# kason-huang/StreamVLN

Measured on AMD Instinct MI355X. Metric: action-steps/sec (8-frame window, StreamVLN-Qwen-1.5), higher is better.
Workload: dtype bf16

## Files before the change

include/streamvln_hip.h:

```cpp
#ifndef STREAMVLN_HIP_H
#define STREAMVLN_HIP_H

#include <stdint.h>

#ifdef __cplusplus
extern "C" {
#endif

typedef struct svln_engine svln_engine;

enum { SVLN_BF16 = 0, SVLN_F32 = 1 };

typedef struct svln_config {
    int32_t v_hidden, v_inter, v_heads, v_layers, v_patch, v_image;
    float v_eps;
    int32_t hidden, layers, q_heads, kv_heads, head_dim, inter, vocab;
    float rope_theta, rms_eps;
    int32_t max_positions;
    int32_t max_envs;
    int32_t max_frames;
    int32_t dtype;
} svln_config;

int svln_create(const svln_config* cfg, int device, svln_engine** out);
// ... 164 lines not shown
int svln_op_gemv_fp8(svln_engine* h, const void* w8, const float* scale, int ldw, const void* x, const void* norm_w, float eps, const void* bias,
                     const void* res, void* y, int N, int K, int epi, int32_t* host_token);
int svln_op_quant_mxfp4(svln_engine* h, const void* w_bf16, int64_t rows, int cols, void* q4, void* e8);
int svln_op_gemv_mxfp4(svln_engine* h, const void* q4, const void* e8, int ldw, const void* x, const void* norm_w, float eps, const void* bias,
                       const void* res, void* y, int N, int K, int epi, int32_t* host_token);
int svln_op_pack_rows(svln_engine* h, const void* w_bf16, int ldw, int64_t rows, int cols, void* packed, void* records, int64_t* fallback_blocks);
int svln_op_unpack_rows(svln_engine* h, const void* packed, const void* records, const void* w_bf16, int ldw, int64_t rows, int cols, void* out);
int svln_op_gemv_packed(svln_engine* h, const void* packed, const void* records, const void* W, int ldw, const void* x, const void* norm_w, float eps,
                        const void* bias, const void* res, void* y, int N, int K, int epi, int32_t* host_token);
int svln_op_gemv_mxfp4_batched(svln_engine* h, const void* q4, const void* e8, int ldw, const void* x, int ldx, const void* bias, const void* res,
                               int ldr, void* y, int ldy, int N, int K, int epi, int B, int32_t* host_tokens);
int svln_op_gemv_mxfp4_batched_argmax_pen(svln_engine* h, const void* q4, const void* e8, int ldw, const void* x, int ldx, int N, int K, int B,
                                          const void* pen_flags, const int32_t* pen_rows, float penalty, int32_t* host_tokens);
int svln_op_gemv_argmax_scores(svln_engine* h, int fmt, const void* W, const void* aux, int ldw, const void* x, int N, int K, const void* pen_flags,
                               float penalty, int32_t* host_token, float* host_logprob);
int svln_op_gemv_argmax_topk(svln_engine* h, int fmt, const void* W, const void* aux, int ldw, const void* x, int N, int K, const void* pen_flags,
                             float penalty, int k, int sampled, float temperature, uint64_t seed, int32_t stream, int32_t draw, int32_t* host_token,
                             float* host_logprob, float* part_val, int32_t* part_idx, float* part_sum, float* part_raw, float* part_max,
                             float* cand_val, int32_t* cand_idx, int32_t* top_ids, float* top_logprobs, int32_t* n_part);
int svln_op_gemv_batched_argmax_topk(svln_engine* h, const void* W, int ldw, const void* x, int ldx, int N, int K, int B, const void* pen_flags,
                                     const int32_t* pen_rows, float penalty, int k, int sampled, float temperature, uint64_t seed, const int32_t* streams,
                                     const int32_t* draws, int32_t* host_tokens, float* host_logprobs, float* cand_val, int32_t* cand_idx,
                                     int32_t* top_ids, float* top_logprobs, int32_t* n_part);
int svln_op_gemm_argmax_topk(svln_engine* h, const void* A, int lda, const void* W, int ldw, int M, int N, int K, const void* pen_flags,
                             const int32_t* pen_rows, float penalty, int k, int sampled, float temperature, uint64_t seed, const int32_t* streams,
                             const int32_t* draws, int32_t* host_tokens, float* host_logprobs, float* cand_val, int32_t* cand_idx, int32_t* top_ids,
                             float* top_logprobs, int32_t* n_part);
int svln_op_truncate(svln_engine* h, const float* cand_val, const int32_t* cand_idx, int B, int n_part, int c, const int32_t* streams,
                     const int32_t* draws, uint64_t seed, float temperature, int32_t top_k, float top_p, float* part_val, int32_t* part_idx,
                     float* part_raw, float* part_max, float* part_sum, int32_t* host_tokens, float* host_logprobs);
int svln_op_gemv_batched_argmax_scores(svln_engine* h, const void* W, int ldw, const void* x, int ldx, const void* norm_w, float eps, int N, int K, int B,
                                       const void* pen_flags, const int32_t* pen_rows, float penalty, int32_t* host_tokens, float* host_logprobs);
int svln_op_gemm_argmax_scores(svln_engine* h, const void* A, int lda, const void* W, int ldw, int M, int N, int K, const void* pen_flags,
                               const int32_t* pen_rows, float penalty, int32_t* host_tokens, float* host_logprobs);
int svln_op_gemv_batched_target(svln_engine* h, const void* W, int ldw, const void* x, int ldx, int N, int K, int B, const int32_t* targets, float inv_t,
                                int32_t* host_tokens, float* host_greedy_logprobs, float* host_logprobs, float* host_slots);
int svln_op_gemm_target(svln_engine* h, const void* A, int lda, const void* W, int ldw, int M, int N, int K, const int32_t* targets, float inv_t,
                        int32_t* host_tokens, float* host_greedy_logprobs, float* host_logprobs, float* host_slots);
int svln_op_read_argmax_partials(svln_engine* h, int rows, int n, float* val, int32_t* idx, float* sum);
int svln_op_gemv_argmax_sample(svln_engine* h, int fmt, const void* W, const void* aux, int ldw, const void* x, int N, int K, const void* pen_flags,
                               float penalty, float temperature, uint64_t seed, int32_t stream, int32_t draw, int32_t* host_token, float* host_logprob);
int svln_op_gemv_batched_argmax_sample(svln_engine* h, const void* W, int ldw, const void* x, int ldx, const void* norm_w, float eps, int N, int K, int B,
                                       const void* pen_flags, const int32_t* pen_rows, float penalty, float temperature, uint64_t seed,
                                       const int32_t* streams, const int32_t* draws, int32_t* host_tokens, float* host_logprobs);
int svln_op_gemm_argmax_sample(svln_engine* h, const void* A, int lda, const void* W, int ldw, int M, int N, int K, const void* pen_flags,
                               const int32_t* pen_rows, float penalty, float temperature, uint64_t seed, const int32_t* streams,
                               const int32_t* draws, int32_t* host_tokens, float* host_logprobs);
int svln_op_gumbel(svln_engine* h, uint64_t seed, int32_t stream, int32_t draw, int32_t n0, int32_t count, float* host_out);
int svln_op_subset_argmax(svln_engine* h, const void* W, int ldw, const void* x, int ldx, int V, int K, int B, const int64_t* ids, int n,
                          const void* pen_flags, const int32_t* pen_rows, float penalty, float temperature, uint64_t seed, const int32_t* streams,
                          const int32_t* draws, int32_t* host_tokens, float* host_logprobs, float* host_y, float* host_dist);
int svln_op_rmsnorm(svln_engine* h, const void* x, const void* g, void* y, int rows, int n, float eps);
int svln_op_layernorm(svln_engine* h, const void* x, const void* g, const void* b, void* y, int rows, int n, float eps);
int svln_op_rmsnorm_tap(svln_engine* h, const void* x, const void* g, void* y, int rows, int n, float eps, int skip_value, void* y2, int y2_row_value,
                        int y2_cap);
int svln_op_rmsnorm_indexed(svln_engine* h, const void* x, int x_rows, const void* g, void* y, const int32_t* src_rows, const int32_t* tap_rows,
                            void* tap, int tap_cap, int rows, int n, float eps);
int svln_op_gather_rows(svln_engine* h, const int32_t* src, int rows, const void* embed, int embed_rows, const void* feats, int feat_rows, void* out,
                        int n, int skip_value);
int svln_op_gather_rows_ragged(svln_engine* h, const int32_t* list, int rows, const void* embed, int embed_rows, void* out, int out_rows, int n);
int svln_op_frame_hash(svln_engine* h, const void* pix_dev, int F, int64_t words_per_frame, uint64_t* out_keys);
int svln_op_attention_llm(svln_engine* h, void* qkv, int ld, int T, int P, const void* ctx_qkv, int ctx_T, void* out, int o_stride,
                          int nsplit);
int svln_op_attention_vit(svln_engine* h, const void* qkv, int ld, int F, void* out, int o_stride);
int svln_op_attention_decode(svln_engine* h, int B, const void* ctx_qkv, int ld, int64_t ctx_rows, const int32_t* pos, const void* qkv_new,
                             void* out, int o_stride);
int svln_op_attention_verify(svln_engine* h, int rows, const void* ctx_qkv, int ld, int ctx_rows, const void* qkv_new, void* out,
                             int o_stride);
int svln_op_attention_verify_multi(svln_engine* h, int n_seq, int rows_max, const void* ctx_qkv, int ld, int ctx_rows, const int32_t* ctx_len,
                                   const void* qkv_new, const int32_t* rows, int share, void* out, int o_stride);
int svln_op_verify_step(svln_engine* h, int rows, const int32_t* fed, const int32_t* cand, int count, int max_new, const int64_t* eos,
                        int n_eos, int32_t* new_count, int32_t* done, int64_t* emitted, int32_t* next_token);
int svln_op_kv_read(svln_engine* h, int env, int start, int n, float* k_out, float* v_out);
int svln_op_kv_pool_read(svln_engine* h, int layer, int start, int n, float* k_out, float* v_out);
int svln_op_kv_page_copy(svln_engine* h, int src_page, const int32_t* dst_pages, int n_dst);
int svln_op_beam_page_gather(svln_engine* h, const int32_t* src_pages, const int32_t* dst_pages, int n);
int svln_op_beam_select(svln_engine* h, int W, int limit, int B, int n_cp, int len_cap, const int32_t* eos, int n_eos, const int32_t* list_ids,
                        const float* list_lps, const int32_t* hdr_in, const float* score_in, const int32_t* ids_in, const float* lps_in,
                        const int32_t* set_pages, int32_t* hdr_out, float* score_out, int32_t* ids_out, float* lps_out, int32_t* tok_b,
                        int32_t* pair_src, int32_t* pair_dst, int32_t* rec);
int svln_op_llm_qkv_rope(svln_engine* h, const void* x, int T, int P, void* q_out, int q_stride, int32_t* fused);
int svln_op_set_pages(svln_engine* h, int env, const int32_t* pages, int n);
int svln_op_fill_attn_state(svln_engine* h, float pool_value, int part_nan);
int svln_op_vit_qkv_attention(svln_engine* h, int layer, const void* x, int F, void* qkv_out, void* attn_out, int o_stride,
                              int force_split, int32_t* packer);
int svln_op_fill_vit_state(svln_engine* h, float pool_value, int part_nan);
int svln_op_vit_kv_read(svln_engine* h, float* k_out, float* v_out);
int svln_op_pool(svln_engine* h, const void* in, void* out, int F);
int svln_op_patchify(svln_engine* h, const float* pix, void* out, int F);

#ifdef __cplusplus
}
#endif
#endif
```

streamvln_amd/_lib.py:

```python
from __future__ import annotations

import ctypes as C
import os

_HERE = os.path.dirname(os.path.abspath(__file__))
LIB_PATH = os.environ.get("SVLN_LIB") or os.path.join(_HERE, "libstreamvln_hip.so")

SVLN_BF16, SVLN_F32 = 0, 1
EPI_NONE, EPI_GELU_TANH, EPI_GELU_ERF, EPI_SWIGLU, EPI_ARGMAX = 0, 1, 2, 3, 4


class SvlnConfig(C.Structure):
    _fields_ = [
        ("v_hidden", C.c_int32), ("v_inter", C.c_int32), ("v_heads", C.c_int32), ("v_layers", C.c_int32),
        ("v_patch", C.c_int32), ("v_image", C.c_int32), ("v_eps", C.c_float),
        ("hidden", C.c_int32), ("layers", C.c_int32), ("q_heads", C.c_int32), ("kv_heads", C.c_int32),
        ("head_dim", C.c_int32), ("inter", C.c_int32), ("vocab", C.c_int32),
        ("rope_theta", C.c_float), ("rms_eps", C.c_float),
        ("max_positions", C.c_int32), ("max_envs", C.c_int32), ("max_frames", C.c_int32), ("dtype", C.c_int32),
    ]


class SvlnTurnArgs(C.Structure):
    _fields_ = [
# ... 140 lines not shown
    "svln_op_decode_layer": (_I, [_P, C.POINTER(SvlnDecodeLayerOp)]),
    "svln_decode_layer_supported": (_I, [_I, _I, _I, _I, _I, _I, _PI32]),
    "svln_decode_layer_walk": (_I, [C.POINTER(SvlnDecodeLayerWalkOp), C.POINTER(SvlnDecodeLayerWalkOp), _I, _I, C.POINTER(SvlnDecodeLayerSlot), _I,
                                    _PI32, _PI64]),
    "svln_set_fp8_decode": (_I, [_P, _I]),
    "svln_set_fp8_gemm": (_I, [_P, _I]),
    "svln_set_fp8_scaled_mfma": (_I, [_P, _I]),
    "svln_set_mxfp4_decode": (_I, [_P, _I]),
    "svln_set_mxfp4_batched": (_I, [_P, _I]),
    "svln_set_packed_decode": (_I, [_P, _I]),
    "svln_packed_stats": (_I, [_P, _PI64, _PI64, _PI64, _PI64]),
    "svln_op_pack_rows": (_I, [_P, _P, _I, _I64, _I, _P, _P, _PI64]),
    "svln_op_unpack_rows": (_I, [_P, _P, _P, _P, _I, _I64, _I, _P]),
    "svln_op_gemv_packed": (_I, [_P, _P, _P, _P, _I, _P, _P, _F, _P, _P, _P, _I, _I, _I, _PI32]),
    "svln_set_speculative": (_I, [_P, _I]),
    "svln_set_draft": (_I, [_P, _I, _PI64, _I]),
    "svln_draft_stats": (_I, [_P, _PI64, _PI64, _PI64, _I]),
    "svln_set_prefill_draft": (_I, [_P, _I]),
    "svln_prefill_draft_stats": (_I, [_P, _PI64, _PI64, _PI64, _I]),
    "svln_set_batch_draft": (_I, [_P, _I]),
    "svln_batch_draft_stats": (_I, [_P, _PI64, _PI64, _PI64, _PI64, _PI64, _I]),
    "svln_set_memory_prune": (_I, [_P, _I]),
    "svln_op_memory_prune": (_I, [_P, _P, _I, _I, _PI32, _PF]),
    "svln_probe_reset": (_I, [_P]),
    "svln_probe_read": (_I, [_P, _PD, _PI64, _PD]),
    "svln_probe_read_prefill": (_I, [_P, _PD, _PI64, _PD, _PD, _PD]),
    "svln_phase_times": (_I, [_P, _PD, _PD, _PD, _I]),
    "svln_set_feature_cache": (_I, [_P, _I]),
    "svln_feature_cache_stats": (_I, [_P, _PI64, _PI64]),
    "svln_op_gemm": (_I, [_P, _P, _I, _P, _I, _P, _I, _P, _P, _I, _I, _I, _I, _I, _I, _I, _I]),
    "svln_op_gemm_norm": (_I, [_P, _P, _I, _P, _I, _P, _I, _P, _P, _I, _P, _P, _P, _F, _I, _I, _I, _I, _PI32]),
    "svln_op_gemm_norm_q8": (_I, [_P, _P, _I, _P, _I, _P, _I, _P, _I, _P, _P, _F, _I, _I, _I, _I, _P, _P, _PI32]),
    "svln_gemm_plan": (_I, [C.POINTER(SvlnGemmProblem), C.POINTER(SvlnGemmPlan)]),
    "svln_op_gemv": (_I, [_P, _P, _I, _P, _P, _F, _P, _P, _P, _I, _I, _I, _PI32]),
    "svln_op_gemm_fp8": (_I, [_P, _P, _P, _I, _P, _P, _I, _P, _I, _P, _P, _I, _I, _I, _I, _I, _I, _I]),
    "svln_op_gemv_batched": (_I, [_P, _P, _I, _P, _I, _P, _F, _P, _P, _I, _P, _I, _I, _I, _I, _I, _PI32]),
    "svln_op_quant_fp8": (_I, [_P, _P, _I64, _I, _P, _P]),
    "svln_op_gemv_fp8": (_I, [_P, _P, _P, _I, _P, _P, _F, _P, _P, _P, _I, _I, _I, _PI32]),
    "svln_op_quant_mxfp4": (_I, [_P, _P, _I64, _I, _P, _P]),
    "svln_op_gemv_mxfp4": (_I, [_P, _P, _P, _I, _P, _P, _F, _P, _P, _P, _I, _I, _I, _PI32]),
    "svln_op_gemv_mxfp4_batched": (_I, [_P, _P, _P, _I, _P, _I, _P, _P, _I, _P, _I, _I, _I, _I, _I, _PI32]),
    "svln_op_gemv_mxfp4_batched_argmax_pen": (_I, [_P, _P, _P, _I, _P, _I, _I, _I, _I, _P, _P, _F, _PI32]),
    "svln_op_gemv_argmax_scores": (_I, [_P, _I, _P, _P, _I, _P, _I, _I, _P, _F, _PI32, _PF]),
    "svln_op_gemv_argmax_topk": (_I, [_P, _I, _P, _P, _I, _P, _I, _I, _P, _F, _I, _I, _F, _U64, _I, _I, _PI32, _PF, _PF, _PI32, _PF, _PF, _PF,
                                      _PF, _PI32, _PI32, _PF, _PI32]),
    "svln_op_gemv_batched_argmax_scores": (_I, [_P, _P, _I, _P, _I, _P, _F, _I, _I, _I, _P, _P, _F, _PI32, _PF]),
    "svln_op_gemm_argmax_scores": (_I, [_P, _P, _I, _P, _I, _I, _I, _I, _P, _P, _F, _PI32, _PF]),
    "svln_op_gemv_argmax_sample": (_I, [_P, _I, _P, _P, _I, _P, _I, _I, _P, _F, _F, _U64, _I, _I, _PI32, _PF]),
    "svln_op_gemv_batched_argmax_sample": (_I, [_P, _P, _I, _P, _I, _P, _F, _I, _I, _I, _P, _P, _F, _F, _U64, _PI32, _PI32, _PI32, _PF]),
    "svln_op_gemm_argmax_sample": (_I, [_P, _P, _I, _P, _I, _I, _I, _I, _P, _P, _F, _F, _U64, _PI32, _PI32, _PI32, _PF]),
    "svln_op_gumbel": (_I, [_P, _U64, _I, _I, _I, _I, _PF]),
    "svln_op_subset_argmax": (_I, [_P, _P, _I, _P, _I, _I, _I, _I, _PI64, _I, _P, _P, _F, _F, _U64, _PI32, _PI32, _PI32, _PF, _PF, _PF]),
    "svln_op_rmsnorm": (_I, [_P, _P, _P, _P, _I, _I, _F]),
    "svln_op_layernorm": (_I, [_P, _P, _P, _P, _P, _I, _I, _F]),
    "svln_op_rmsnorm_tap": (_I, [_P, _P, _P, _P, _I, _I, _F, _I, _P, _I, _I]),
    "svln_op_rmsnorm_indexed": (_I, [_P, _P, _I, _P, _P, _PI32, _PI32, _P, _I, _I, _I, _F]),
    "svln_op_gather_rows": (_I, [_P, _PI32, _I, _P, _I, _P, _I, _P, _I, _I]),
    "svln_op_gather_rows_ragged": (_I, [_P, _PI32, _I, _P, _I, _P, _I, _I]),
    "svln_op_frame_hash": (_I, [_P, _P, _I, _I64, C.POINTER(C.c_uint64)]),
    "svln_op_attention_llm": (_I, [_P, _P, _I, _I, _I, _P, _I, _P, _I, _I]),
    "svln_op_attention_vit": (_I, [_P, _P, _I, _I, _P, _I]),
    "svln_op_attention_decode": (_I, [_P, _I, _P, _I, _I64, _PI32, _P, _P, _I]),
    "svln_op_attention_verify": (_I, [_P, _I, _P, _I, _I, _P, _P, _I]),
    "svln_op_attention_verify_multi": (_I, [_P, _I, _I, _P, _I, _I, _PI32, _P, _PI32, _I, _P, _I]),
    "svln_op_verify_step": (_I, [_P, _I, _PI32, _PI32, _I, _I, _PI64, _I, _PI32, _PI32, _PI64, _PI32]),
    "svln_op_kv_read": (_I, [_P, _I, _I, _I, _PF, _PF]),
    "svln_op_llm_qkv_rope": (_I, [_P, _P, _I, _I, _P, _I, _PI32]),
    "svln_op_set_pages": (_I, [_P, _I, _PI32, _I]),
    "svln_op_fill_attn_state": (_I, [_P, _F, _I]),
    "svln_op_vit_qkv_attention": (_I, [_P, _I, _P, _I, _P, _P, _I, _I, _PI32]),
    "svln_op_fill_vit_state": (_I, [_P, _F, _I]),
    "svln_op_vit_kv_read": (_I, [_P, _PF, _PF]),
    "svln_op_pool": (_I, [_P, _P, _P, _I]),
    "svln_op_patchify": (_I, [_P, _P, _P, _I]),
}

_lib = None


def load():
    global _lib
    if _lib is None:
        if not os.path.exists(LIB_PATH):
            raise RuntimeError(f"{LIB_PATH} is missing: build it with streamvln_amd/csrc/build.sh "
                               f"(or __graft_entry__.build()); there is no fallback path")
        import torch
        lib = C.CDLL(LIB_PATH)
        for name, (res, args) in SIGNATURES.items():
            fn = getattr(lib, name)
            fn.restype, fn.argtypes = res, args
        _lib = lib
    return _lib


class SvlnError(RuntimeError):
    pass


def check(rc: int):
    if rc != 0:
        raise SvlnError(load().svln_last_error().decode("utf-8", "replace"))
```

streamvln_amd/csrc/attention.hip:

```cpp
#include <type_traits>

#include "common.h"
#include "kernels.h"

namespace svln {

namespace {

template <typename T, int HD> struct AttnGeom {
    static constexpr int EPC = Elt<T>::PER_CHUNK;
    static constexpr int HDC = (((HD + EPC - 1) / EPC) + 1) & ~1;
    static constexpr int HDP = HDC * EPC;
    static constexpr int DT = (HD + 31) / 32;
    static constexpr int VROWS = DT * 32;
    static constexpr int VC = 64 / EPC;
    static constexpr bool KSWZ = (HDC % 16) == 0;
    static constexpr int KROW = (KSWZ ? HDC : HDC + 1) * 16;
    static constexpr int K_TILE_BYTES = 64 * KROW;
    static constexpr int V_TILE_BYTES = VROWS * VC * 16;
};

SVLN_DEV float fast_exp2(float x) { return __builtin_amdgcn_exp2f(x); }

template <typename G> SVLN_DEV int k_off(int row, int c) {
    return row * G::KROW + ((G::KSWZ ? (c ^ (row & 15)) : c) << 4);
}
SVLN_DEV int v_off_f32(int row, int c) { return row * 256 + ((c ^ (row & 15)) << 4); }
SVLN_DEV int v_off_bf16(int row, int unit) { return row * 128 + ((unit ^ ((row >> 1) & 15)) << 3); }

template <int OFF> SVLN_DEV void lds_read_b64(uint2& v, unsigned addr) { asm volatile("ds_read_b64 %0, %1 offset:%2" : "=v"(v) : "v"(addr), "n"(OFF)); }
template <int N> SVLN_DEV void lds_wait(uint2& a, uint2& b) { asm volatile("s_waitcnt lgkmcnt(%2)" : "+v"(a), "+v"(b) : "n"(N)); }
template <int I, int N, typename F> SVLN_DEV void static_for(F&& f) {
    if constexpr (I < N) { f(std::integral_constant<int, I>{}); static_for<I + 1, N>(f); }
}

template <typename T, int HD, int WAVES, int KG = 1, int PF = 1>
__global__ __launch_bounds__(WAVES * 64 * KG, (KG == 1 && WAVES == 4 && sizeof(T) == 2) ? 2 : 1) void attn_kernel(AttnArgs p) {
    using G = AttnGeom<T, HD>;
    constexpr int NT = WAVES * 64;
    constexpr int EPC = G::EPC;
    extern __shared__ __attribute__((aligned(16))) char smem[];
    const int kg = KG == 1 ? 0 : (int)threadIdx.x / NT;
    char* sK = smem + kg * (G::K_TILE_BYTES + G::V_TILE_BYTES);
    char* sV = sK + G::K_TILE_BYTES;

    const int tid = KG == 1 ? (int)threadIdx.x : (int)threadIdx.x - kg * NT, lane = tid & 63, wave = tid >> 6;
    const int r = lane & 31, h = lane >> 5;
    const int kh = blockIdx.y;
    const int frame = kh / p.hpf, head0 = (kh % p.hpf) * p.G;
    const int kt0 = blockIdx.z * p.tiles_per_split + kg;
    const int page0 = p.page_table ? p.page_table[kt0] : kt0;
    const int kv_len = p.dyn_kv_len ? *p.dyn_kv_len : p.kv_len;
    const int P = p.dyn_kv_len ? kv_len - p.T : p.P;
    const int rows_total = p.T * p.G;
    const int rho = (blockIdx.x * WAVES + wave) * 32 + r;
    const bool valid = rho < rows_total;
    const int qi = valid ? rho / p.G : 0;
    const int qg = valid ? rho - qi * p.G : 0;
    const int qpos = P + qi;

    uint4 qf[G::HDC / 2];
    {
        const T* qrow = (const T*)p.Q + (size_t)(frame * p.T + qi) * p.q_stride + (size_t)(head0 + qg) * HD;
#pragma unroll
        for (int s = 0; s < G::HDC / 2; ++s) {
            const int e0 = (2 * s + h) * EPC;
            qf[s] = (valid && e0 < HD) ? *(const uint4*)(qrow + e0) : zero_chunk();
        }
    }
    int tiles = (kv_len + 63) >> 6;
    if (p.causal) {
        const int last_row = min((int)(blockIdx.x + 1) * WAVES * 32, rows_total) - 1;
        const int last_pos = P + last_row / p.G;
        tiles = min(tiles, (last_pos >> 6) + 1);
    }
    const int kt_begin = blockIdx.z * p.tiles_per_split + kg;
    const int kt_end = min(tiles, (int)blockIdx.z * p.tiles_per_split + p.tiles_per_split);
    const int n_iter = (kt_end - (int)blockIdx.z * p.tiles_per_split + KG - 1) / KG;

    const float scale2 = p.scale * 1.4426950408889634f;
    f32x16 O[G::DT];
#pragma unroll
    for (int d = 0; d < G::DT; ++d)
#pragma unroll
        for (int e = 0; e < 16; ++e) O[d][e] = 0.0f;
    float m = -INFINITY, l = 0.0f;

    const size_t k_page_stride = (size_t)p.n_kv_total * 64 * G::HDP * sizeof(T);
    const size_t v_page_stride = (size_t)p.n_kv_total * G::VROWS * 64 * sizeof(T);

    constexpr bool PFK = WAVES == 4 || (KG > 1 && PF >= 1), PFV = WAVES == 4 || (KG > 1 && PF == 1);
    constexpr int KTOT = 64 * G::HDC, VTOT = G::VROWS * G::VC, B = WAVES == 1 ? 4 : 8;
    constexpr int KL = (KTOT + NT - 1) / NT, VL = (VTOT + NT - 1) / NT;
    uint4 pk[PFK ? KL : 1], pv[PFV ? VL : 1];
    auto tile_ptrs = [&](int kt, const char*& gk, const char*& gv) {
        const int pg = kt == kt0 ? page0 : (p.page_table ? p.page_table[kt] : kt);
        gk = (const char*)p.Kpool + (size_t)pg * k_page_stride + (size_t)kh * 64 * G::HDP * sizeof(T);
        gv = (const char*)p.Vpool + (size_t)pg * v_page_stride + (size_t)kh * G::VROWS * 64 * sizeof(T);
    };
    auto put_k = [&](int q, const uint4& v) {
        const int row = q / G::HDC, c = q - row * G::HDC;
        *(uint4*)(sK + k_off<G>(row, c)) = v;
    };
    auto put_v = [&](int q, const uint4& v) {
        const int row = q / G::VC, c = q - row * G::VC;
        if (sizeof(T) == 4) {
            *(uint4*)(sV + v_off_f32(row, c)) = v;
        } else {
            *(uint2*)(sV + v_off_bf16(row, 2 * c)) = make_uint2(v.x, v.y);
            *(uint2*)(sV + v_off_bf16(row, 2 * c + 1)) = make_uint2(v.z, v.w);
        }
    };
    auto load_regs = [&](int kt) {
        const char *gk, *gv;
        tile_ptrs(kt, gk, gv);
        if (PFK) {
#pragma unroll
            for (int u = 0; u < KL; ++u) {
                const int q = tid + u * NT;
                pk[u] = q < KTOT ? *(const uint4*)(gk + (size_t)q * 16) : zero_chunk();
            }
        }
        if (PFV) {
#pragma unroll
            for (int u = 0; u < VL; ++u) {
                const int q = tid + u * NT;
                pv[u] = q < VTOT ? *(const uint4*)(gv + (size_t)q * 16) : zero_chunk();
            }
        }
    };
    if (PFK && kt_begin < kt_end) load_regs(kt_begin);
// ... 18 lines not shown
                    for (int u = 0; u < B; ++u) {
                        const int q = tid + (b0 + u) * NT;
                        t[u] = (b0 + u < KL && q < KTOT) ? *(const uint4*)(gK + (size_t)q * 16) : zero_chunk();
                    }
#pragma unroll
                    for (int u = 0; u < B; ++u) {
                        const int q = tid + (b0 + u) * NT;
                        if (b0 + u < KL && q < KTOT) put_k(q, t[u]);
                    }
                }
            }
            if (PFV) {
#pragma unroll
                for (int u = 0; u < VL; ++u) {
                    const int q = tid + u * NT;
                    if (q < VTOT) put_v(q, pv[u]);
                }
            } else {
#pragma unroll
                for (int b0 = 0; b0 < VL; b0 += B) {
                    uint4 t[B];
#pragma unroll
                    for (int u = 0; u < B; ++u) {
                        const int q = tid + (b0 + u) * NT;
                        t[u] = (b0 + u < VL && q < VTOT) ? *(const uint4*)(gV + (size_t)q * 16) : zero_chunk();
                    }
#pragma unroll
                    for (int u = 0; u < B; ++u) {
                        const int q = tid + (b0 + u) * NT;
                        if (b0 + u < VL && q < VTOT) put_v(q, t[u]);
                    }
                }
            }
        }
        __syncthreads();
        if (PFK && kt + KG < kt_end) load_regs(kt + KG);
        if (act) {

        f32x16 S[2];
#pragma unroll
        for (int j = 0; j < 2; ++j)
#pragma unroll
            for (int e = 0; e < 16; ++e) S[j][e] = 0.0f;
#pragma unroll
        for (int s = 0; s < G::HDC / 2; ++s) {
#pragma unroll
            for (int j = 0; j < 2; ++j) {
                const uint4 a = *(const uint4*)(sK + k_off<G>(j * 32 + r, 2 * s + h));
                mma_chunk<T>(a, qf[s], S[j]);
            }
        }

        const int tile_last_key = kt * 64 + 63;
        const bool need_mask = tile_last_key >= kv_len || (p.causal && tile_last_key > P + (int)(blockIdx.x * WAVES * 32) / p.G);
        if (need_mask) {
#pragma unroll
            for (int j = 0; j < 2; ++j)
#pragma unroll
                for (int e = 0; e < 16; ++e) {
                    const int key = kt * 64 + j * 32 + acc_row(e, lane);
                    if (!(key < kv_len && (!p.causal || key <= qpos))) S[j][e] = -INFINITY;
                }
        }
        float mloc = -INFINITY;
#pragma unroll
        for (int j = 0; j < 2; ++j)
#pragma unroll
            for (int e = 0; e < 16; ++e) mloc = fmaxf(mloc, S[j][e]);
        mloc = fmaxf(mloc, __shfl_xor(mloc, 32, 64)) * scale2;
        const float mnew = fmaxf(m, mloc);
        float alpha = 1.0f, psum = 0.0f;
        if (mnew == -INFINITY) {
#pragma unroll
            for (int j = 0; j < 2; ++j)
#pragma unroll
                for (int e = 0; e < 16; ++e) S[j][e] = 0.0f;
        } else {
            alpha = fast_exp2(m - mnew);
#pragma unroll
            for (int j = 0; j < 2; ++j)
#pragma unroll
                for (int e = 0; e < 16; ++e) {
                    const float pv = fast_exp2(fmaf(S[j][e], scale2, -mnew));
                    S[j][e] = pv;
                    psum += pv;
                }
        }
        l = l * alpha + psum;
        m = mnew;
        if (__builtin_amdgcn_ballot_w64(alpha != 1.0f) != 0) {
#pragma unroll
            for (int d = 0; d < G::DT; ++d)
#pragma unroll
                for (int e = 0; e < 16; ++e) O[d][e] *= alpha;
        }

        if (sizeof(T) == 2) {
            const unsigned sv0 = (unsigned)(size_t)(__attribute__((address_space(3))) char*)sV + r * 128;
            const int xr = (r >> 1) & 15;
#pragma unroll
            for (int ks = 0; ks < 4; ++ks) {
                const int j = ks >> 1, b0 = 8 * (ks & 1);
                const unsigned alo = sv0 + (((4 * ks + h) ^ xr) << 3), ahi = sv0 + (((4 * ks + 2 + h) ^ xr) << 3);
                uint2 vlo[G::DT], vhi[G::DT];
                static_for<0, G::DT>([&](auto dc) {
                    constexpr int d = decltype(dc)::value;
                    lds_read_b64<d * 4096>(vlo[d], alo);
// ... 8 lines not shown
                                                                   __builtin_bit_cast(bf16x8, pf), O[d], 0, 0, 0);
                });
            }
        } else {
#pragma unroll
            for (int j = 0; j < 2; ++j)
#pragma unroll
                for (int g4 = 0; g4 < 4; ++g4) {
#pragma unroll
                    for (int d = 0; d < G::DT; ++d) {
                        const uint4 a = *(const uint4*)(sV + v_off_f32(d * 32 + r, j * 8 + 2 * g4 + h));
                        O[d] = __builtin_amdgcn_mfma_f32_32x32x2f32(__uint_as_float(a.x), S[j][4 * g4 + 0], O[d], 0, 0, 0);
                        O[d] = __builtin_amdgcn_mfma_f32_32x32x2f32(__uint_as_float(a.y), S[j][4 * g4 + 1], O[d], 0, 0, 0);
                        O[d] = __builtin_amdgcn_mfma_f32_32x32x2f32(__uint_as_float(a.z), S[j][4 * g4 + 2], O[d], 0, 0, 0);
                        O[d] = __builtin_amdgcn_mfma_f32_32x32x2f32(__uint_as_float(a.w), S[j][4 * g4 + 3], O[d], 0, 0, 0);
                    }
                }
        }
        }
        __syncthreads();
    }

    l += __shfl_xor(l, 32, 64);
    if constexpr (KG > 1) {
        constexpr int ROWS = WAVES * 32, OP = HD + ATTN_PART_PAD;
        float* sML = (float*)smem;
        float* sFin = (float*)(smem + KG * ROWS * 8);
        float* sO = (float*)(smem + (KG + 1) * ROWS * 8);
        const int rowl = wave * 32 + r;
        if (h == 0) *(float2*)(sML + (kg * ROWS + rowl) * 2) = make_float2(m, l);
        __syncthreads();
        float M = -INFINITY;
#pragma unroll
        for (int g = 0; g < KG; ++g) M = fmaxf(M, sML[(g * ROWS + rowl) * 2]);
        float L = 0.0f;
#pragma unroll
        for (int g = 0; g < KG; ++g) {
            const float2 ml = *(const float2*)(sML + (g * ROWS + rowl) * 2);
            L += ml.x == -INFINITY ? 0.0f : ml.y * fast_exp2(ml.x - M);
        }
        if (kg == 0 && h == 0) *(float2*)(sFin + rowl * 2) = make_float2(M, L);
        const float f = m == -INFINITY ? 0.0f : fast_exp2(m - M);
        float* od = sO + (size_t)(kg * ROWS + rowl) * OP;
#pragma unroll
        for (int d = 0; d < G::DT; ++d)
#pragma unroll
            for (int e4 = 0; e4 < 4; ++e4) {
                const int dd = d * 32 + acc_row(e4 * 4, lane);
                if (dd < HD) *(float4*)(od + dd) = make_float4(O[d][4 * e4] * f, O[d][4 * e4 + 1] * f, O[d][4 * e4 + 2] * f, O[d][4 * e4 + 3] * f);
            }
        __syncthreads();
        for (int q = threadIdx.x; q < ROWS * (HD / 4); q += NT * KG) {
            const int row = q / (HD / 4), c4 = q - row * (HD / 4);
            const int rho_o = blockIdx.x * ROWS + row;
            if (rho_o >= rows_total) continue;
            float4 acc = *(const float4*)(sO + (size_t)row * OP + c4 * 4);
#pragma unroll
            for (int g = 1; g < KG; ++g) {
                const float4 v = *(const float4*)(sO + (size_t)(g * ROWS + row) * OP + c4 * 4);
                acc.x += v.x; acc.y += v.y; acc.z += v.z; acc.w += v.w;
            }
            const float2 fin = *(const float2*)(sFin + row * 2);
            if (p.nsplit > 1) {
                float* dst = p.part + (((size_t)blockIdx.z * p.n_kv_total + kh) * p.rows_pad + rho_o) * OP;
                *(float4*)(dst + c4 * 4) = acc;
                if (c4 == 0) { dst[HD] = fin.x; dst[HD + 1] = fin.y; }
                continue;
            }
            const float inv = fin.y > 0.0f ? 1.0f / fin.y : 0.0f;
            const int qi_o = rho_o / p.G, qg_o = rho_o - qi_o * p.G;
            T* orow = (T*)p.O + (size_t)(frame * p.T + qi_o) * p.o_stride + (size_t)(head0 + qg_o) * HD + c4 * 4;
            if (sizeof(T) == 2) *(uint2*)orow = make_uint2(pack_bf16x2(acc.x * inv, acc.y * inv), pack_bf16x2(acc.z * inv, acc.w * inv));
            else *(float4*)orow = make_float4(acc.x * inv, acc.y * inv, acc.z * inv, acc.w * inv);
        }
        return;
    }
    if (!valid) return;

    if (p.nsplit > 1) {
        float* dst = p.part + (((size_t)blockIdx.z * p.n_kv_total + kh) * p.rows_pad + rho) * (HD + ATTN_PART_PAD);
#pragma unroll
        for (int d = 0; d < G::DT; ++d)
#pragma unroll
            for (int e4 = 0; e4 < 4; ++e4) {
                const int dd = d * 32 + acc_row(e4 * 4, lane);
                if (dd < HD) *(float4*)(dst + dd) = make_float4(O[d][4 * e4], O[d][4 * e4 + 1], O[d][4 * e4 + 2], O[d][4 * e4 + 3]);
            }
        if (h == 0) { dst[HD] = m; dst[HD + 1] = l; }
        return;
    }

    const float inv = l > 0.0f ? 1.0f / l : 0.0f;
    T* orow = (T*)p.O + (size_t)(frame * p.T + qi) * p.o_stride + (size_t)(head0 + qg) * HD;
#pragma unroll
    for (int d = 0; d < G::DT; ++d)
#pragma unroll
        for (int e4 = 0; e4 < 4; ++e4) {
            const int dd = d * 32 + acc_row(e4 * 4, lane);
            if (dd < HD) {
                if (sizeof(T) == 2) {
                    *(uint2*)(orow + dd) = make_uint2(pack_bf16x2(O[d][4 * e4] * inv, O[d][4 * e4 + 1] * inv),
                                                      pack_bf16x2(O[d][4 * e4 + 2] * inv, O[d][4 * e4 + 3] * inv));
                } else {
                    *(float4*)(orow + dd) = make_float4(O[d][4 * e4] * inv, O[d][4 * e4 + 1] * inv, O[d][4 * e4 + 2] * inv,
                                                        O[d][4 * e4 + 3] * inv);
                }
            }
        }
}

template <typename T>
__global__ __launch_bounds__(256) void attn_decode_kernel(AttnArgs p) {
    using G = AttnGeom<T, 128>;
    constexpr int EPC = G::EPC, NT = 256;
    extern __shared__ __attribute__((aligned(16))) char smem[];
    if (p.skip && *p.skip) return;
    char* sK = smem;
    char* sV = smem + G::K_TILE_BYTES;
    const int tid = threadIdx.x, lane = tid & 63, wave = tid >> 6;
    const int r = lane & 31, h = lane >> 5;
    const int kh = blockIdx.x, z = blockIdx.y, env = blockIdx.z;
    const int kt0 = z * p.tiles_per_split;
    const int* page_table = p.slots ? p.slots[env].page_table : p.page_table;
    const int page0 = page_table[kt0];
    const int pos = p.slots ? p.slots[env].pos : *p.dyn_pos;
    const T* qkv_row = (const T*)p.Q + (size_t)env * p.q_stride;
    const int kv_len = pos + 1;
    const int tiles = (kv_len + 63) >> 6;
    if (kt0 >= tiles) return;
    const int kt_end = min(tiles, kt0 + p.tiles_per_split);
    const size_t k_page_stride = (size_t)p.n_kv_total * 64 * 128 * sizeof(T);
    const bool valid = r < p.G;

// ... 304 lines not shown
#pragma unroll
            for (int ks = 0; ks < 4; ++ks) {
                const int j = ks >> 1, b0 = 8 * (ks & 1);
                const uint4 pf = make_uint4(pack_bf16x2(S[j][b0 + 0], S[j][b0 + 1]), pack_bf16x2(S[j][b0 + 2], S[j][b0 + 3]),
                                            pack_bf16x2(S[j][b0 + 4], S[j][b0 + 5]), pack_bf16x2(S[j][b0 + 6], S[j][b0 + 7]));
                const uint2 lo = *(const uint2*)(sV + v_off_bf16(row, 4 * ks + h));
                const uint2 hi = *(const uint2*)(sV + v_off_bf16(row, 4 * ks + 2 + h));
                O = __builtin_amdgcn_mfma_f32_32x32x16_bf16(__builtin_bit_cast(bf16x8, make_uint4(lo.x, lo.y, hi.x, hi.y)),
                                                            __builtin_bit_cast(bf16x8, pf), O, 0, 0, 0);
            }
        } else {
#pragma unroll
            for (int j = 0; j < 2; ++j)
#pragma unroll
                for (int g4 = 0; g4 < 4; ++g4) {
                    const uint4 a = *(const uint4*)(sV + v_off_f32(row, j * 8 + 2 * g4 + h));
                    O = __builtin_amdgcn_mfma_f32_32x32x2f32(__uint_as_float(a.x), S[j][4 * g4 + 0], O, 0, 0, 0);
                    O = __builtin_amdgcn_mfma_f32_32x32x2f32(__uint_as_float(a.y), S[j][4 * g4 + 1], O, 0, 0, 0);
                    O = __builtin_amdgcn_mfma_f32_32x32x2f32(__uint_as_float(a.z), S[j][4 * g4 + 2], O, 0, 0, 0);
                    O = __builtin_amdgcn_mfma_f32_32x32x2f32(__uint_as_float(a.w), S[j][4 * g4 + 3], O, 0, 0, 0);
                }
        }
        __syncthreads();
    }
    l += __shfl_xor(l, 32, 64);
    if (!valid) return;
    float* dst = part + (((size_t)z * p.n_kv_total + kh) * p.rows_pad + r) * (128 + ATTN_PART_PAD);
#pragma unroll
    for (int e4 = 0; e4 < 4; ++e4)
        *(float4*)(dst + wave * 32 + acc_row(e4 * 4, lane)) = make_float4(O[4 * e4], O[4 * e4 + 1], O[4 * e4 + 2], O[4 * e4 + 3]);
    if (wave == 0 && h == 0) { dst[128] = m; dst[129] = l; }
}

template <typename T>
__global__ __launch_bounds__(256) void attn_verify_kernel(AttnArgs p) {
    extern __shared__ __attribute__((aligned(16))) char smem[];
    if (p.skip && *p.skip) return;
    attn_verify_body<T>(p, p.page_table, *p.dyn_pos, *p.dyn_rows, (const T*)p.Q, p.part, smem);
}
template <typename T>
__global__ __launch_bounds__(256) void attn_verify_multi_kernel(AttnArgs p) {
    extern __shared__ __attribute__((aligned(16))) char smem[];
    const int s = blockIdx.z;
    const DecodeSlot sl = p.slots[s];
    attn_verify_body<T>(p, sl.page_table, sl.pos, sl.pad, (const T*)p.Q + (size_t)s * p.T * p.q_stride, p.part + (size_t)s * p.part_bstride, smem);
}

template <typename T, int HD, bool VERIFY = false, bool MULTI = false>
__global__ __launch_bounds__(256) void attn_combine_kernel(AttnArgs p) {
    __shared__ float wsh_all[4][64];
    if (p.skip && *p.skip) return;
    const int wave = threadIdx.x >> 6, lane = threadIdx.x & 63;
    float* wsh = wsh_all[wave];
    const int rho = blockIdx.x * (blockDim.x >> 6) + wave, kh = blockIdx.y, env = blockIdx.z;
    int kv_len;
    if constexpr (VERIFY && MULTI) {
        const int rows = min(p.slots[env].pad, p.T);
        if (rho >= rows * p.G) return;
        kv_len = p.slots[env].pos + rows;
    } else if constexpr (VERIFY) {
        const int rows = min(*p.dyn_rows, p.T);
        if (rho >= rows * p.G) return;
        kv_len = *p.dyn_pos + rows;
    } else {
        if (rho >= p.T * p.G) return;
        kv_len = p.slots ? p.slots[env].pos + 1 : (p.dyn_kv_len ? *p.dyn_kv_len : p.kv_len);
    }
    const int tiles = (kv_len + 63) >> 6;
    const int nsplit = min(min(p.nsplit, 64), (tiles + p.tiles_per_split - 1) / p.tiles_per_split);
    const size_t split_stride = (size_t)p.n_kv_total * p.rows_pad * (HD + ATTN_PART_PAD);
    const float* base = p.part + (size_t)env * p.part_bstride + ((size_t)kh * p.rows_pad + rho) * (HD + ATTN_PART_PAD);
    float mz = -INFINITY, lz = 0.0f;
    if (lane < nsplit) { mz = base[lane * split_stride + HD]; lz = base[lane * split_stride + HD + 1]; }
    const float mstar = wave_max(mz);
    const float w = mz == -INFINITY ? 0.0f : fast_exp2(mz - mstar);
    const float lsum = wave_sum(w * lz);
    wsh[lane] = w;
    __builtin_amdgcn_wave_barrier();
    float o0 = 0.0f, o1 = 0.0f;
    for (int z = 0; z < nsplit; ++z) {
        const float* pz = base + z * split_stride;
        const float wz = wsh[z];
        if (lane < HD) o0 += wz * pz[lane];
        if (lane + 64 < HD) o1 += wz * pz[lane + 64];
    }
    const float inv = lsum > 0.0f ? 1.0f / lsum : 0.0f;
    const int qi = rho / p.G, qg = rho - qi * p.G;
    const int frame = kh / p.hpf, head0 = (kh % p.hpf) * p.G;
    T* orow = (T*)p.O + (size_t)(frame * p.T + qi + (MULTI ? env * p.T : env)) * p.o_stride + (size_t)(head0 + qg) * HD;
    if (lane < HD) orow[lane] = from_f32<T>(o0 * inv);
    if (lane + 64 < HD) orow[lane + 64] = from_f32<T>(o1 * inv);
}

template <typename T, int HD, int WAVES> void launch_attn_t(hipStream_t s, const AttnArgs& a) {
    using G = AttnGeom<T, HD>;
    const int rows = a.T * a.G;
    dim3 grid((rows + WAVES * 32 - 1) / (WAVES * 32), a.n_kv_total, a.nsplit), block(WAVES * 64);
    const size_t lds = G::K_TILE_BYTES + G::V_TILE_BYTES;
    hipLaunchKernelGGL((attn_kernel<T, HD, WAVES>), grid, block, lds, s, a);
}
template <typename T> struct VitGroups { static constexpr int KG = sizeof(T) == 2 ? 4 : 3; static constexpr int PF = sizeof(T) == 2 ? 1 : 0; };
template <typename T, int HD, int KG_> struct GroupGeom {
    using G = AttnGeom<T, HD>;
    static constexpr int WAVES = 2, ROWS = WAVES * 32;
    static constexpr int KG = KG_;
    static constexpr size_t TILES = (size_t)KG * (G::K_TILE_BYTES + G::V_TILE_BYTES);
    static constexpr size_t MERGE = (size_t)(KG + 1) * ROWS * 8 + (size_t)KG * ROWS * (HD + ATTN_PART_PAD) * 4;
    static constexpr size_t LDS = TILES > MERGE ? TILES : MERGE;
};
template <typename T, int HD, int KG, int PF> void launch_attn_groups(hipStream_t s, const AttnArgs& a) {
    using GG = GroupGeom<T, HD, KG>;
    const int rows = a.T * a.G;
    dim3 grid((rows + GG::ROWS - 1) / GG::ROWS, a.n_kv_total, a.nsplit), block(GG::WAVES * 64 * GG::KG);
    hipLaunchKernelGGL((attn_kernel<T, HD, GG::WAVES, GG::KG, PF>), grid, block, GG::LDS, s, a);
}

}

template <typename T> void launch_attention(hipStream_t s, const AttnArgs& a, int head_dim, int waves) {
    if (head_dim == 128 && waves == 1 && a.fuse_rope_append && a.T == 1) {
        using G = AttnGeom<T, 128>;
        hipLaunchKernelGGL((attn_decode_kernel<T>), dim3(a.n_kv_total, a.nsplit, a.batch > 0 ? a.batch : 1), dim3(256), G::K_TILE_BYTES + G::V_TILE_BYTES, s, a);
        return;
    }
    if (a.key_groups > 1) {
        if (head_dim != 72 || a.key_groups != attn_key_groups<T>(head_dim))
            throw std::runtime_error("attention: key groups are built for head_dim 72 with key_groups == attn_key_groups<T>(72)");
        launch_attn_groups<T, 72, VitGroups<T>::KG, VitGroups<T>::PF>(s, a);
        return;
    }
    if (head_dim == 128) {
        if (waves == 1) launch_attn_t<T, 128, 1>(s, a); else launch_attn_t<T, 128, 4>(s, a);
    } else if (head_dim == 72) {
        if (waves == 1) launch_attn_t<T, 72, 1>(s, a); else launch_attn_t<T, 72, 4>(s, a);
    }
}
template <typename T> void launch_attention_combine(hipStream_t s, const AttnArgs& a, int head_dim) {
    const int rows = a.T * a.G, rpw = rows >= 256 ? 4 : 1;
    dim3 grid((rows + rpw - 1) / rpw, a.n_kv_total, a.batch > 0 ? a.batch : 1), block(64 * rpw);
    if (head_dim == 128) hipLaunchKernelGGL((attn_combine_kernel<T, 128>), grid, block, 0, s, a);
    else if (head_dim == 72) hipLaunchKernelGGL((attn_combine_kernel<T, 72>), grid, block, 0, s, a);
}
template <typename T> void launch_attention_verify(hipStream_t s, const AttnArgs& a) {
    using G = AttnGeom<T, 128>;
    if (!(a.T >= 1 && a.T * a.G <= 32 && a.dyn_rows && a.dyn_pos && a.page_table && a.rows_pad >= 32 && a.fuse_rope_append))
        throw std::runtime_error("verify attention: 1 <= rows, rows * G <= 32, device row count / position and a page table");
    hipLaunchKernelGGL((attn_verify_kernel<T>), dim3(a.n_kv_total, a.nsplit), dim3(256), G::K_TILE_BYTES + G::V_TILE_BYTES, s, a);
    hipLaunchKernelGGL((attn_combine_kernel<T, 128, true>), dim3(a.T * a.G, a.n_kv_total), dim3(64), 0, s, a);
}
template <typename T> void launch_attention_verify_multi(hipStream_t s, const AttnArgs& a) {
    using G = AttnGeom<T, 128>;
    if (!(a.T >= 1 && a.T * a.G <= 32 && a.slots && a.batch >= 1 && a.batch <= 8 && a.rows_pad >= 32 && a.fuse_rope_append && a.nsplit >= 1 &&
          a.part_bstride >= (size_t)a.nsplit * a.n_kv_total * a.rows_pad * (128 + ATTN_PART_PAD)))
        throw std::runtime_error("batched verify attention: 1 <= rows, rows * G <= 32, 1 .. 8 sequences with device slots, a partial stride that holds one sequence's splits");
    hipLaunchKernelGGL((attn_verify_multi_kernel<T>), dim3(a.n_kv_total, a.nsplit, a.batch), dim3(256), G::K_TILE_BYTES + G::V_TILE_BYTES, s, a);
    hipLaunchKernelGGL((attn_combine_kernel<T, 128, true, true>), dim3(a.T * a.G, a.n_kv_total, a.batch), dim3(64), 0, s, a);
}
template <typename T, int HD, int WAVES> static void attn_attr() {
    using G = AttnGeom<T, HD>;
    set_max_lds((const void*)attn_kernel<T, HD, WAVES>, G::K_TILE_BYTES + G::V_TILE_BYTES);
}
void attention_init_attrs() {
    set_max_lds((const void*)attn_decode_kernel<float>, AttnGeom<float, 128>::K_TILE_BYTES + AttnGeom<float, 128>::V_TILE_BYTES);
    set_max_lds((const void*)attn_verify_kernel<float>, AttnGeom<float, 128>::K_TILE_BYTES + AttnGeom<float, 128>::V_TILE_BYTES);
    set_max_lds((const void*)attn_verify_multi_kernel<float>, AttnGeom<float, 128>::K_TILE_BYTES + AttnGeom<float, 128>::V_TILE_BYTES);
    attn_attr<bf16, 128, 1>(); attn_attr<bf16, 128, 4>(); attn_attr<bf16, 72, 1>(); attn_attr<bf16, 72, 4>();
    attn_attr<float, 128, 1>(); attn_attr<float, 128, 4>(); attn_attr<float, 72, 1>(); attn_attr<float, 72, 4>();
    set_max_lds((const void*)attn_kernel<bf16, 72, 2, VitGroups<bf16>::KG, VitGroups<bf16>::PF>, GroupGeom<bf16, 72, VitGroups<bf16>::KG>::LDS);
    set_max_lds((const void*)attn_kernel<float, 72, 2, VitGroups<float>::KG, VitGroups<float>::PF>, GroupGeom<float, 72, VitGroups<float>::KG>::LDS);
}
template <typename T> int attn_key_groups(int head_dim) { return head_dim == 72 ? VitGroups<T>::KG : 1; }
template int attn_key_groups<bf16>(int);
template int attn_key_groups<float>(int);
template void launch_attention<bf16>(hipStream_t, const AttnArgs&, int, int);
template void launch_attention<float>(hipStream_t, const AttnArgs&, int, int);
template void launch_attention_verify<bf16>(hipStream_t, const AttnArgs&);
template void launch_attention_verify<float>(hipStream_t, const AttnArgs&);
template void launch_attention_verify_multi<bf16>(hipStream_t, const AttnArgs&);
template void launch_attention_verify_multi<float>(hipStream_t, const AttnArgs&);
template void launch_attention_combine<bf16>(hipStream_t, const AttnArgs&, int);
template void launch_attention_combine<float>(hipStream_t, const AttnArgs&, int);

}
```

streamvln_amd/csrc/engine.hip:

```cpp
#include <hip/hip_runtime.h>

#include <algorithm>
#include <cmath>
#include <cstdio>
#include <cstdlib>
#include <cstring>
#include <stdexcept>
#include <string>
#include <unordered_map>
#include <vector>

#include "../../include/streamvln_hip.h"
#include "common.h"
#include "gemm_plan.h"
#include "kernels.h"

namespace svln {

static thread_local std::string g_err;

#define HIP_CHECK(x)                                                                                   \
    do {                                                                                               \
        hipError_t e_ = (x);                                                                           \
        if (e_ != hipSuccess)                                                                          \
// ... 124 lines not shown
    virtual void op_kv_pool_read(int layer, int start, int n, float* k_out, float* v_out) = 0;
    virtual void sync() = 0;
    virtual void set_graph(int enable) = 0;
    virtual void set_decode_persistent(int enable) = 0;
    virtual void probe_decode_layer(int layer, unsigned long long* out, int max_wgs, int32_t* n_wgs) = 0;
    virtual void op_decode_layer(const svln_decode_layer_op& q) = 0;
    virtual void set_fp8_decode(int enable) = 0;
    virtual void set_fp8_gemm(int enable) = 0;
    virtual void set_fp8_scaled_mfma(int enable) = 0;
    virtual void set_mxfp4_decode(int enable) = 0;
    virtual void set_mxfp4_batched(int enable) = 0;
    virtual void set_speculative(int rows) = 0;
    virtual void set_draft(int env, const int64_t* ids, int n) = 0;
    virtual void draft_stats(int64_t* verify_passes, int64_t* tokens_from_verify, int64_t* single_steps, int reset) = 0;
    virtual void set_prefill_draft(int on) = 0;
    virtual void prefill_draft_stats(int64_t* rides, int64_t* tokens_from_rides, int64_t* rows_fed, int reset) = 0;
    virtual void set_batch_draft(int on) = 0;
    virtual void batch_draft_stats(int64_t* rides, int64_t* tokens_from_rides, int64_t* rows_fed, int64_t* iterations, int64_t* single_rows, int reset) = 0;
    virtual void op_attention_verify(int rows, const void* ctx, int ld, int ctx_rows, const void* qkv_new, void* out, int o_stride) = 0;
    virtual void op_attention_verify_multi(int S, int T, const void* ctx, int ld, int ctx_rows, const int32_t* ctx_len, const void* qkv_new,
                                           const int32_t* rows, int share, void* out, int o_stride) = 0;
    virtual void op_verify_step(int rows, const int32_t* fed, const int32_t* cand, int count, int max_new, const int64_t* eos, int n_eos,
                                int32_t* new_count, int32_t* done, int64_t* emitted, int32_t* next_token) = 0;
    virtual bool op_gemm_fp8(const GemmArgs& a) = 0;
    virtual void set_memory_prune(int keep) = 0;
    virtual void op_memory_prune(const void* m, int n_rows, int keep, int32_t* out_idx, float* out_score) = 0;
    virtual void probe_reset() = 0;
    virtual void probe_read(double* ms, int64_t* launches, double* bytes) = 0;
    virtual void phase_times(double* v, double* p, double* d, int reset) = 0;
    virtual void probe_read_prefill(double* ms, int64_t* n, double* rows, double* flops, double* wbytes) = 0;
    virtual void set_feature_cache(int cap) = 0;
    virtual void feature_cache_stats(int64_t* hits, int64_t* misses) = 0;
    virtual bool op_gemm(const GemmArgs& a) = 0;
    virtual void op_gemv(GemvArgs a, int32_t* host_token) = 0;
    virtual void op_gemv_batched(GemvBatchArgs a, int32_t* host_tokens) = 0;
    virtual void op_gemv_mxfp4_batched(GemvMx4BatchArgs a, int32_t* host_tokens) = 0;
    virtual void op_quant_fp8(const void* w, int64_t rows, int cols, void* w8, float* scale) = 0;
    virtual void set_packed_decode(int enable) = 0;
    virtual void packed_stats(int64_t* packed_bytes, int64_t* bf16_bytes, int64_t* blocks, int64_t* fallback_blocks) = 0;
    virtual void op_pack_rows(const void* w, int ldw, int64_t rows, int cols, void* packed, void* rec, int64_t* fallback_blocks) = 0;
    virtual void op_unpack_rows(const void* packed, const void* rec, const void* w, int ldw, int64_t rows, int cols, void* out) = 0;
    virtual void op_quant_mxfp4(const void* w, int64_t rows, int cols, void* q4, uint8_t* e8) = 0;
    virtual void op_rmsnorm(const void* x, const void* g, void* y, int rows, int n, float eps) = 0;
    virtual void op_layernorm(const void* x, const void* g, const void* b, void* y, int rows, int n, float eps) = 0;
    virtual void op_rmsnorm_tap(const void* x, const void* g, void* y, int rows, int n, float eps, int skip_value, void* y2, int y2_row_value,
                                int y2_cap) = 0;
    virtual void op_rmsnorm_indexed(const void* x, int x_rows, const void* g, void* y, const int32_t* src_rows, const int32_t* tap_rows, void* tap,
                                    int tap_cap, int rows, int n, float eps) = 0;
    virtual void op_gather_rows(const int32_t* src, int rows, const void* embed, int embed_rows, const void* feats, int feat_rows, void* out, int n,
                                int skip_value) = 0;
    virtual void op_gather_rows_ragged(const int32_t* list, int rows, const void* embed, int embed_rows, void* out, int out_rows, int n) = 0;
    virtual void op_frame_hash(const void* pix, int F, int64_t words_per_frame, uint64_t* out_keys) = 0;
    virtual void op_attention_llm(void* qkv, int ld, int T, int P, const void* ctx, int ctx_T, void* out, int o_stride, int nsplit) = 0;
    virtual void op_attention_vit(const void* qkv, int ld, int F, void* out, int o_stride) = 0;
    virtual void op_attention_decode(int B, const void* ctx, int ld, int64_t ctx_rows, const int32_t* pos, const void* qkv_new, void* out,
                                     int o_stride) = 0;
    virtual void op_kv_read(int env, int start, int n, float* k_out, float* v_out) = 0;
    virtual void op_llm_qkv_rope(const void* x, int T, int P, void* q_out, int q_stride, int32_t* fused) = 0;
    virtual void op_set_pages(int env, const int32_t* pages, int n) = 0;
    virtual void op_fill_attn_state(float pool_value, int part_nan) = 0;
    virtual void op_vit_qkv_attention(int layer, const void* x, int F, void* qkv_out, void* attn_out, int o_stride, int force_split,
                                      int32_t* packer) = 0;
    virtual void op_fill_vit_state(float pool_value, int part_nan) = 0;
    virtual void op_vit_kv_read(float* k_out, float* v_out) = 0;
    virtual void op_pool(const void* in, void* out, int F) = 0;
    virtual void op_patchify(const float* pix, void* out, int F) = 0;
};

template <typename T>
class Engine : public EngineBase {
public:
    svln_config c;
    int device;
    hipStream_t st = nullptr;
    std::vector<void*> allocs;
    std::unordered_map<std::string, Slot> slots;

    int Hv, Iv, vheads, vhd, side, S, kp, oside, otok, H, I, nq, nkv, qkv_dim, V;
    int vhdp, vvrows, vtiles;
    int pages_per_env, pages_total;

    struct VLayer { T *ln1_w, *ln1_b, *qkv_w, *qkv_b, *out_w, *out_b, *ln2_w, *ln2_b, *fc1_w, *fc1_b, *fc2_w, *fc2_b; };
    struct Q8 { uint8_t* q = nullptr; float* s = nullptr; };
    struct Q4 { uint8_t* q = nullptr; uint8_t* e8 = nullptr; };
    struct P12 { uint8_t* pk = nullptr; uint8_t* rec = nullptr; unsigned* fb = nullptr; const T* w = nullptr; int64_t rows = 0; int cols = 0; };
    struct LLayer { T *in_norm, *qkv_w, *qkv_b, *o_w, *post_norm, *gu_w, *down_w, *kpool, *vpool; Q8 qkv8, o8, gu8, down8; Q4 qkv4, o4, gu4, down4; P12 gu12, down12; };
    P12 lm_head12; bool p12_on = false;
    std::unordered_map<const void*, P12*> p12_of;
    Q8 lm_head8; bool fp8_on = false, fp8_built = false;
    Q4 lm_head4; bool mx4_on = false, mx4_built = false;
    bool mx4b_on = false;
    bool fp8_scaled_on = false;
    bool fp8_gemm_on = false; uint8_t* act8 = nullptr; float* act8_scale = nullptr;
    T *patch_w, *patch_b, *pos_emb, *proj0_w, *proj0_b, *proj2_w, *proj2_b, *embed, *final_norm, *lm_head;
    std::vector<VLayer> vl;
    std::vector<LLayer> ll;

    float* pix = nullptr;
    T *patches, *vx, *vn, *vqkv, *vattn, *vh, *vkpool, *vvpool, *proj_h, *proj_o, *feats;
    int n_feat_frames = 0;
    int* tap_idx; float* tap_w;
    T *x, *xn, *qkv, *attn, *hbuf, *hid_tap, *head_xn;
    float* gemm_ws = nullptr; size_t gemm_ws_elems = 0; void* zero_line = nullptr;
    float* inv_freq; float* rope_tab;
    float* attn_part; size_t attn_part_elems = 0; int nsplit_max, tiles_per_split;
    float* part_val; int* part_idx; int* d_token; float* d_top2;
    GenCtl* d_ctl;
    GenCtl* h_ctl = nullptr;
    int *d_eos = nullptr, *d_out_ids = nullptr, *h_out_ids = nullptr; std::vector<int> eos_cached; bool eos_valid = false;
    static constexpr int RUN_AHEAD = 4;
    static constexpr int MAXB = 8;
    static constexpr int batched_mfma_min = 4;
    DecodeSlot* d_slots = nullptr; DecodeSlot* h_slots = nullptr; int* d_tok_b = nullptr; int* h_tok_b = nullptr;
    float* part_val_b = nullptr; int* part_idx_b = nullptr; T* last_rows = nullptr; int n_generated_b[MAXB] = {0};
    int* d_src; int* h_src;
    int prune_keep = 0; float *prune_partial = nullptr, *prune_mean = nullptr, *prune_score = nullptr; int *d_sel = nullptr, *h_sel = nullptr;
    int* h_token;
    float* h_top2;
    bool scores_on = false;
    float *part_sum = nullptr, *part_sum_b = nullptr, *d_scores = nullptr, *h_scores = nullptr, *d_score_b = nullptr, *h_score_b = nullptr;
    float* row_scale_b = nullptr;
    int topk = 0;
    float *cand_val = nullptr, *d_topl = nullptr, *h_topl = nullptr; int *cand_idx = nullptr, *d_topi = nullptr, *h_topi = nullptr;
    std::vector<int32_t> last_topi; std::vector<float> last_topl; int last_topk = 0; bool last_topk_valid = false;
    float *cand_val_b = nullptr, *d_topl_b = nullptr, *h_topl_b = nullptr; int *cand_idx_b = nullptr, *d_topi_b = nullptr, *h_topi_b = nullptr;
    std::vector<std::vector<int32_t>> gb_topi; std::vector<std::vector<float>> gb_topl; int gb_topk = 0; bool gb_topk_valid = false;
    void ensure_topk_buffers() {
        if (cand_val) return;
        const size_t rows = (size_t)c.max_positions + 8;
        cand_val = dalloc<float>((size_t)2048 * TOPK_C); cand_idx = dalloc<int>((size_t)2048 * TOPK_C);
        d_topi = dalloc<int>(rows * TOPK_C, true); d_topl = dalloc<float>(rows * TOPK_C, true);
        HIP_CHECK(hipHostMalloc((void**)&h_topi, rows * TOPK_C * sizeof(int)));
        HIP_CHECK(hipHostMalloc((void**)&h_topl, rows * TOPK_C * sizeof(float)));
        cand_val_b = dalloc<float>((size_t)HEAD_ROWS * 2048 * TOPK_C); cand_idx_b = dalloc<int>((size_t)HEAD_ROWS * 2048 * TOPK_C);
        d_topi_b = dalloc<int>((size_t)(HEAD_ROWS + MAXB) * TOPK_C, true); d_topl_b = dalloc<float>((size_t)(HEAD_ROWS + MAXB) * TOPK_C, true);
        HIP_CHECK(hipHostMalloc((void**)&h_topi_b, (size_t)(HEAD_ROWS + MAXB) * TOPK_C * sizeof(int)));
        HIP_CHECK(hipHostMalloc((void**)&h_topl_b, (size_t)(HEAD_ROWS + MAXB) * TOPK_C * sizeof(float)));
    }
    std::vector<float> last_scores; bool last_scores_valid = false;
    static constexpr int SMP_ROWS = 64 + 8;
    bool smp_on = false; float smp_inv_t = 1.0f; uint64_t smp_seed = 0;
    float *part_raw = nullptr, *part_max = nullptr, *part_raw_b = nullptr, *part_max_b = nullptr;
    int *d_smp = nullptr, *h_smp = nullptr;
    std::vector<int> env_draws;
    int trunc_k = 0; float trunc_p = 1.0f;
    float *tr_val = nullptr, *tr_raw = nullptr, *tr_max = nullptr, *tr_sum = nullptr, *tr_val_b = nullptr, *tr_raw_b = nullptr, *tr_max_b = nullptr, *tr_sum_b = nullptr;
    int *tr_idx = nullptr, *tr_idx_b = nullptr;
    void ensure_trunc_buffers() {
        ensure_topk_buffers();
        if (tr_val) return;
        tr_val = dalloc<float>(TOPK_C); tr_raw = dalloc<float>(TOPK_C); tr_max = dalloc<float>(TOPK_C); tr_sum = dalloc<float>(TOPK_C); tr_idx = dalloc<int>(TOPK_C);
        const size_t nb = (size_t)SMP_ROWS * TOPK_C;
        tr_val_b = dalloc<float>(nb); tr_raw_b = dalloc<float>(nb); tr_max_b = dalloc<float>(nb); tr_sum_b = dalloc<float>(nb); tr_idx_b = dalloc<int>(nb);
    }
    bool top2_sampled = false;
    SampleArgs smp_args(const int* stream, const int* draw, const int* count, float* raw, float* mx) const {
        SampleArgs q; q.stream = stream; q.draw = draw; q.count = count; q.inv_t = smp_inv_t;
        q.seed_lo = (uint32_t)smp_seed; q.seed_hi = (uint32_t)(smp_seed >> 32); q.part_raw = raw; q.part_max = mx; return q;
// ... 175 lines not shown
            p12_on = true;
        }

        const size_t rv = (size_t)c.max_frames * S;
        pix = dalloc<float>((size_t)c.max_frames * 3 * c.v_image * c.v_image);
        patches = dalloc<T>(rv * kp); vx = dalloc<T>(rv * Hv); vn = dalloc<T>(rv * Hv); vqkv = dalloc<T>(rv * 3 * Hv);
        vattn = dalloc<T>(rv * Hv); vh = dalloc<T>(rv * Iv);
        vkpool = dalloc<T>((size_t)vtiles * c.max_frames * vheads * PAGE * vhdp, true);
        vvpool = dalloc<T>((size_t)vtiles * c.max_frames * vheads * vvrows * PAGE, true);
        proj_h = dalloc<T>(rv * H); proj_o = dalloc<T>(rv * H);
        feats = dalloc<T>((size_t)c.max_frames * otok * H);
        {
            std::vector<int> ti(2 * oside); std::vector<float> tw(2 * oside);
            const double scale = (double)side / (double)oside;
            for (int d = 0; d < oside; ++d) {
                double src = (d + 0.5) * scale - 0.5; if (src < 0) src = 0;
                int i0 = (int)std::floor(src); if (i0 > side - 1) i0 = side - 1;
                int i1 = i0 + 1 < side ? i0 + 1 : side - 1;
                float l1 = (float)(src - i0);
                ti[2 * d] = i0; ti[2 * d + 1] = i1; tw[2 * d] = 1.0f - l1; tw[2 * d + 1] = l1;
            }
            tap_idx = dalloc<int>(2 * oside); tap_w = dalloc<float>(2 * oside);
            HIP_CHECK(hipMemcpy(tap_idx, ti.data(), ti.size() * sizeof(int), hipMemcpyHostToDevice));
            HIP_CHECK(hipMemcpy(tap_w, tw.data(), tw.size() * sizeof(float), hipMemcpyHostToDevice));
        }
        const size_t rt = (size_t)c.max_positions;
        x = dalloc<T>(rt * H); xn = dalloc<T>(rt * H); qkv = dalloc<T>(rt * qkv_dim); attn = dalloc<T>(rt * qd); hbuf = dalloc<T>(rt * I);
        hid_tap = dalloc<T>((size_t)HID_TAP_ROWS * H);
        head_xn = dalloc<T>((size_t)H);
        {
            size_t widest = (size_t)(qkv_dim > 3 * Hv ? qkv_dim : 3 * Hv);
            if ((size_t)Iv > widest) widest = Iv;
            size_t rows = (size_t)c.max_frames * S > 768 ? (size_t)c.max_frames * S : 768;
            gemm_ws_elems = 8 * rows * widest;
            if (gemm_ws_elems > (size_t)64 << 20) gemm_ws_elems = (size_t)64 << 20;
            gemm_ws = dalloc<float>(gemm_ws_elems);
            zero_line = dalloc<char>(256, true);
        }
        {
            std::vector<float> f(64);
            for (int j = 0; j < 64; ++j) f[j] = 1.0f / powf(c.rope_theta, (float)(2 * j) / 128.0f);
            inv_freq = dalloc<float>(64);
            HIP_CHECK(hipMemcpy(inv_freq, f.data(), 64 * sizeof(float), hipMemcpyHostToDevice));
            rope_tab = dalloc<float>((size_t)c.max_positions * 128);
            launch_rope_table(st, rope_tab, inv_freq, c.max_positions);
        }
        tiles_per_split = 1;
        while ((pages_per_env + tiles_per_split - 1) / tiles_per_split > 64) ++tiles_per_split;
        nsplit_max = (pages_per_env + tiles_per_split - 1) / tiles_per_split;
        {
            constexpr int PW = 128 + ATTN_PART_PAD;
            const size_t dec = (size_t)MAXB * nsplit_max * nkv * 32 * PW, pre = (size_t)8 * nkv * PREFILL_SPLIT_ROWS * PW;
            attn_part_elems = dec > pre ? dec : pre;
            attn_part = dalloc<float>(attn_part_elems);
        }
        part_val = dalloc<float>(2048); part_idx = dalloc<int>(2048); part_sum = dalloc<float>(2048);
        d_scores = dalloc<float>((size_t)c.max_positions + 8, true); d_score_b = dalloc<float>(HEAD_ROWS + MAXB, true);
        part_sum_b = dalloc<float>((size_t)HEAD_ROWS * 2048); row_scale_b = dalloc<float>(MAXB, true);
        static_assert(SMP_ROWS == HEAD_ROWS + MAXB, "SMP_ROWS");
        part_raw = dalloc<float>(2048); part_max = dalloc<float>(2048);
        part_raw_b = dalloc<float>((size_t)HEAD_ROWS * 2048); part_max_b = dalloc<float>((size_t)HEAD_ROWS * 2048);
        d_smp = dalloc<int>(2 * SMP_ROWS, true);
        HIP_CHECK(hipHostMalloc((void**)&h_smp, 2 * SMP_ROWS * sizeof(int)));
        HIP_CHECK(hipHostMalloc((void**)&h_scores, ((size_t)c.max_positions + 8) * sizeof(float)));
        HIP_CHECK(hipHostMalloc((void**)&h_score_b, (HEAD_ROWS + MAXB) * sizeof(float)));
        d_token = dalloc<int>(4, true); d_top2 = dalloc<float>(4, true);
        d_ctl = (GenCtl*)dalloc<int>(sizeof(GenCtl) / sizeof(int), true);
        d_eos = dalloc<int>((size_t)(V > 16 ? V : 16)); d_out_ids = dalloc<int>((size_t)c.max_positions + 8);
        HIP_CHECK(hipHostMalloc((void**)&h_ctl, sizeof(GenCtl)));
        HIP_CHECK(hipHostMalloc((void**)&h_out_ids, ((size_t)c.max_positions + 8) * sizeof(int)));
        d_slots = dalloc<DecodeSlot>(MAXB, true); d_tok_b = dalloc<int>(HEAD_ROWS + MAXB, true);
        part_val_b = dalloc<float>((size_t)HEAD_ROWS * 2048); part_idx_b = dalloc<int>((size_t)HEAD_ROWS * 2048);
        last_rows = dalloc<T>((size_t)HEAD_ROWS * H);
        HIP_CHECK(hipHostMalloc((void**)&h_slots, MAXB * sizeof(DecodeSlot)));
        HIP_CHECK(hipHostMalloc((void**)&h_tok_b, (HEAD_ROWS + MAXB) * sizeof(int)));
        d_head_src = dalloc<int>(2 * HEAD_ROWS + 2 * RIDE_PAIRS, true); d_head_tap = d_head_src + HEAD_ROWS; d_ride_list = d_head_src + 2 * HEAD_ROWS;
        HIP_CHECK(hipHostMalloc((void**)&h_head_src, (2 * HEAD_ROWS + 2 * RIDE_PAIRS) * sizeof(int)));
        h_head_tap = h_head_src + HEAD_ROWS; h_ride_list = h_head_src + 2 * HEAD_ROWS;
        d_src = dalloc<int>(rt);
        HIP_CHECK(hipHostMalloc((void**)&h_src, rt * sizeof(int)));
        HIP_CHECK(hipHostMalloc((void**)&h_token, 16));
        HIP_CHECK(hipHostMalloc((void**)&h_top2, 16));
        envs.resize(c.max_envs);
        env_draws.assign(c.max_envs, 0);
        graphs.resize(c.max_envs);
        for (auto& e : envs) {
            e.embeds = dalloc<T>(rt * H);
            e.d_pages = dalloc<int>(pages_per_env, true);
            e.pages.assign(pages_per_env, 0);
        }
        for (int p = pages_total - 1; p >= 0; --p) free_pages.push_back(p);
        for (int i = 0; i < 5; ++i) HIP_CHECK(hipEventCreate(&ph_ev[i]));
        HIP_CHECK(init_kernel_attributes());
        HIP_CHECK(hipStreamSynchronize(st));
    }

    ~Engine() override {
        int prev = -1;
        (void)hipGetDevice(&prev);
        (void)hipSetDevice(device);
        (void)hipStreamSynchronize(st);
        drop_graphs();
        if (d_rgb) (void)hipFree(d_rgb);
        for (auto& t : rs_tabs) for (void* p : t.bufs) (void)hipFree(p);
        for (int i = 0; i < 2; ++i) {
            if (h_rgb[i]) (void)hipHostFree(h_rgb[i]);
            if (h2d_ev[i]) (void)hipEventDestroy(h2d_ev[i]);
        }
        for (auto& pr : pp_ring) { if (pr.a) (void)hipEventDestroy(pr.a); if (pr.b) (void)hipEventDestroy(pr.b); }
        if (src_ev) (void)hipEventDestroy(src_ev);
        for (auto ev : ring_ev) (void)hipEventDestroy(ev);
        if (ring_host) (void)hipHostFree(ring_host);
        for (auto e : probe_ev) (void)hipEventDestroy(e);
        for (auto e : pprobe_ev) (void)hipEventDestroy(e);
        for (int i = 0; i < 5; ++i) (void)hipEventDestroy(ph_ev[i]);
        (void)hipHostFree(h_ctl); (void)hipHostFree(h_out_ids); (void)hipHostFree(h_scores); (void)hipHostFree(h_score_b);
        if (h_topi) (void)hipHostFree(h_topi);
        if (h_topl) (void)hipHostFree(h_topl);
        if (h_topi_b) (void)hipHostFree(h_topi_b);
        if (h_topl_b) (void)hipHostFree(h_topl_b);
        if (h_smp) (void)hipHostFree(h_smp);
        if (h_fork_dst) (void)hipHostFree(h_fork_dst);
        if (h_alp) (void)hipHostFree(h_alp);
        if (h_alp_b) (void)hipHostFree(h_alp_b);
        if (h_giveup) (void)hipHostFree(h_giveup);
        if (h_hash) (void)hipHostFree(h_hash);
        for (void* p : allocs) (void)hipFree(p);
        (void)hipHostFree(h_src); (void)hipHostFree(h_token); (void)hipHostFree(h_top2);
        if (h_sel) (void)hipHostFree(h_sel);
        (void)hipHostFree(h_slots); (void)hipHostFree(h_tok_b);
        if (h_head_src) (void)hipHostFree(h_head_src);
        if (bf_host_i) (void)hipHostFree(bf_host_i);
        if (h_cfeed) (void)hipHostFree(h_cfeed);
        if (h_cslots) (void)hipHostFree(h_cslots);
        if (bf_host_f) (void)hipHostFree(bf_host_f);
        if (bf_host_alp) (void)hipHostFree(bf_host_alp);
        if (h_draft) (void)hipHostFree(h_draft);
        if (h_vctl) (void)hipHostFree(h_vctl);
        if (h_pen_rows) (void)hipHostFree(h_pen_rows);
        if (h_pen_ids) (void)hipHostFree(h_pen_ids);
        (void)hipStreamDestroy(st);
        if (prev >= 0 && prev != device) (void)hipSetDevice(prev);
    }

    Slot& slot(const char* name) {
        auto it = slots.find(name);
        REQUIRE(it != slots.end(), std::string("unknown tensor: ") + name);
        return it->second;
    }
    void synth_tensor(const char* name, uint64_t seed_t, float hw, float base) override {
        Slot& s = slot(name);
        before_weight_write("svln_synth_tensor");
        launch_synth<T>(st, s.dst, s.ld, s.rows, s.cols, s.map, seed_t, hw, base);
        s.filled = true;
        after_weight_write(s);
    }
    void before_weight_write(const char* who) {
        refuse_while_jobs(who);
        refuse_while_group(who);
    }
    void after_weight_write(const Slot& s) {
        p12_encode(s.dst);
        requantise(s.dst);
// ... 397 lines not shown
            if (t == IMAGE_TOKEN) {
                REQUIRE(img < n_feat_frames, "more <image> tokens than encoded frames");
                for (int j = 0; j < otok; ++j) src.push_back(-(1 + img * otok + j));
                ++img;
            } else if (t == MEMORY_TOKEN) {
                REQUIRE(n_memory > 0 && mem_used == 0, "<memory> token without (or with repeated) memory frames");
                const int nm = n_memory * otok;
                if (prune_keep > 0 && prune_keep < nm) {
                    run_memory_prune(feats + (size_t)frame_base * otok * H, nm, prune_keep);
                    for (int j = 0; j < prune_keep; ++j) src.push_back(-(1 + frame_base * otok + h_sel[j]));
                } else {
                    for (int j = 0; j < nm; ++j) src.push_back(-(1 + frame_base * otok + j));
                }
                mem_used = 1;
            } else {
                REQUIRE(t >= 0 && t < V, "token id out of range");
                src.push_back((int)t);
            }
        }
        if (src.size() > lim) src.resize(lim);
        REQUIRE((int)src.size() <= cap, "inputs_embeds exceeds max_positions");
        const int rows = (int)src.size();
        std::memcpy(h_src, src.data(), (size_t)rows * sizeof(int));
        HIP_CHECK(hipMemcpyAsync(d_src, h_src, rows * sizeof(int), hipMemcpyHostToDevice, st));
        launch_gather_rows<T>(st, d_src, embed, feats, e.embeds + (size_t)e.n_embeds * H, rows, H);
        if (!src_ev) HIP_CHECK(hipEventCreateWithFlags(&src_ev, hipEventDisableTiming));
        HIP_CHECK(hipEventRecord(src_ev, st));
        src_pending = true;
        e.n_embeds += rows;
    }

    AttnArgs llm_attn_args(const LLayer& L, const Env& e, const void* q, int ld, void* out, int o_stride, int Tn, int P, int kv_len,
                           bool decode) {
        AttnArgs a; std::memset(&a, 0, sizeof(a));
        a.Q = q; a.q_stride = ld; a.O = out; a.o_stride = o_stride; a.Kpool = L.kpool; a.Vpool = L.vpool; a.page_table = e.d_pages;
        a.n_kv_total = nkv; a.hpf = nkv; a.G = nq / nkv; a.T = Tn; a.P = P; a.kv_len = kv_len; a.scale = 1.0f / sqrtf(128.0f);
        a.part = attn_part; a.rows_pad = 32;
        if (decode) {
            a.causal = 0; a.dyn_kv_len = &d_ctl->kv_len; a.nsplit = nsplit_max; a.tiles_per_split = tiles_per_split;
            a.fuse_rope_append = 1; a.rope_tab = rope_tab; a.dyn_pos = &d_ctl->pos; a.nq_heads = nq; a.skip = &d_ctl->done;
        } else {
            a.causal = 1; a.dyn_kv_len = nullptr; a.nsplit = 1; a.tiles_per_split = pages_per_env;
            const int rows = Tn * a.G, wgs = ((rows + 127) / 128) * nkv, tiles = (kv_len + PAGE - 1) / PAGE;
            if (rows <= PREFILL_SPLIT_ROWS && wgs < 128 && tiles >= 4) {
                int ns = (256 + wgs - 1) / wgs;
                if (ns > 8) ns = 8;
                if (ns > tiles / 2) ns = tiles / 2;
                if (ns > 1) { a.nsplit = ns; a.tiles_per_split = (tiles + ns - 1) / ns; a.rows_pad = PREFILL_SPLIT_ROWS; }
            }
        }
        return a;
    }

    struct Seg { Env* e; int P, Tn, off; int n_draft = 0; };
    RopeKvArgs rope_kv_args(const LLayer& L, const Seg& g) {
        RopeKvArgs r; r.qkv = qkv + (size_t)g.off * qkv_dim; r.ld = qkv_dim; r.Kpool = L.kpool; r.Vpool = L.vpool; r.rope_tab = rope_tab;
        r.nq = nq; r.nkv = nkv; r.dyn_pos = nullptr; r.page_table = g.e->d_pages; r.T = g.Tn; r.P = g.P;
        return r;
    }
    bool prefill_qkv(const LLayer& L, int M, const Seg* single) {
        GemmArgs aq = gemm_args(xn, H, L.qkv_w, H, qkv, qkv_dim, L.qkv_b, nullptr, 0, 0, M, qkv_dim, H, EPI_NONE);
        RopeKvArgs r0;
        if (single) { r0 = rope_kv_args(L, *single); aq.rope = &r0; }
        return llm_gemm(aq, L.qkv8);
    }
    void prefill_rope_append(const LLayer& L, const Seg& g) { launch_rope_kv<T>(st, rope_kv_args(L, g)); }
    void prefill_rows(const std::vector<Seg>& segs, int M, int n_dec = 0, int n_ragged = 0) {
        const int qd = nq * 128;
        for (const Seg& g : segs) {
            HIP_CHECK(hipMemcpyAsync(x + (size_t)g.off * H, g.e->embeds + (size_t)g.P * H, (size_t)(g.Tn - g.n_draft) * H * sizeof(T), hipMemcpyDeviceToDevice, st));
            if (g.n_draft > 0 && n_ragged == 0)
                launch_gather_rows<T>(st, d_draft, embed, feats, x + (size_t)(g.off + g.Tn - g.n_draft) * H, g.n_draft, H);
        }
        launch_gather_rows_ragged<T>(st, d_ride_list, embed, x, n_ragged, H);
        bool xn_ready = false;
        const bool taps = layer_taps_on && segs.size() == 1 && n_dec == 0;
        for (int i = 0; i < c.layers; ++i) {
            const LLayer& L = ll[i];
            const bool probing = taps && i == probe_layer;
            if (probing) { probe_copy(0, x, M); probe_rows = M; }
            if (!xn_ready) launch_rmsnorm<T>(st, x, L.in_norm, xn, M, H, c.rms_eps);
            if (probing) probe_copy(6, xn, M);
            const bool roped = prefill_qkv(L, M, segs.size() == 1 && n_dec == 0 ? &segs[0] : nullptr);
            if (n_dec > 0) decode_attention(batched_decode_attn_args(L, n_dec));
            for (const Seg& g : segs) {
                T* q_g = qkv + (size_t)g.off * qkv_dim;
                if (!roped) prefill_rope_append(L, g);
                AttnArgs a = llm_attn_args(L, *g.e, q_g, qkv_dim, attn + (size_t)g.off * qd, qd, g.Tn, g.P, g.P + g.Tn, false);
                launch_attention<T>(st, a, 128, 4);
                if (a.nsplit > 1) launch_attention_combine<T>(st, a, 128);
            }
            GemmArgs ao = gemm_args(attn, qd, L.o_w, qd, x, H, nullptr, x, H, 0, M, H, qd, EPI_NONE);
            ao.norm_w = L.post_norm; ao.norm_out = xn; ao.norm_eps = c.rms_eps;
            if (probing) { probe_copy(2, attn, M); probe_copy(7, qkv, M); }
            if (!llm_gemm(ao, L.o8)) launch_rmsnorm<T>(st, x, L.post_norm, xn, M, H, c.rms_eps);
            if (probing) { probe_copy(3, x, M); probe_copy(4, xn, M); }
            const bool pp = i == 0 && probe_on && M <= 256 && n_dec == 0 && pprobe_used + 2 <= pprobe_ev.size();
            if (pp) HIP_CHECK(hipEventRecord(pprobe_ev[pprobe_used], st));
            llm_gemm(gemm_args(xn, H, L.gu_w, H, hbuf, I, nullptr, nullptr, 0, 0, M, 2 * I, H, EPI_SWIGLU), L.gu8);
            if (pp) { HIP_CHECK(hipEventRecord(pprobe_ev[pprobe_used + 1], st)); pprobe_used += 2; pprobe_rows += M; }
            if (probing) probe_copy(5, hbuf, M);
            GemmArgs ad = gemm_args(hbuf, I, L.down_w, I, x, H, nullptr, x, H, 0, M, H, I, EPI_NONE);
            if (i + 1 < c.layers) { ad.norm_w = ll[i + 1].in_norm; ad.norm_out = xn; ad.norm_eps = c.rms_eps; }
            xn_ready = llm_gemm(ad, L.down8);
            if (taps) {
                HIP_CHECK(hipMemcpyAsync(layer_tap + (size_t)i * H, x + (size_t)(M - 1) * H, (size_t)H * sizeof(T), hipMemcpyDeviceToDevice, st));
                if (probing) probe_copy(1, x, M);
            }
        }
    }
    AttnArgs decode_attn_args(const LLayer& L, const Env& e) { return llm_attn_args(L, e, qkv, qkv_dim, attn, nq * 128, 1, 0, 0, true); }
    AttnArgs batched_decode_attn_args(const LLayer& L, int B) {
        AttnArgs a = decode_attn_args(L, envs[0]);
        a.page_table = nullptr; a.dyn_kv_len = nullptr; a.dyn_pos = nullptr; a.skip = nullptr;
        a.slots = d_slots; a.batch = B; a.part_bstride = (size_t)nsplit_max * nkv * 32 * (128 + ATTN_PART_PAD);
        return a;
    }
    AttnArgs verify_attn_args(const LLayer& L, const Env& e, int rows) {
        AttnArgs a = decode_attn_args(L, e);
        a.T = rows; a.dyn_rows = d_vctl + 1;
        return a;
    }
    AttnArgs verify_multi_attn_args(const LLayer& L, int S, int rows, int kv_max, const DecodeSlot* slots = nullptr) {
        AttnArgs a = batched_decode_attn_args(L, S);
        a.T = rows;
        const int tiles = (kv_max + PAGE - 1) / PAGE;
        a.nsplit = std::max(1, std::min(nsplit_max, (tiles + tiles_per_split - 1) / tiles_per_split));
        if (slots) a.slots = slots;
        return a;
    }
    void decode_attention(const AttnArgs& a) {
        launch_attention<T>(st, a, 128, 1);
        launch_attention_combine<T>(st, a, 128);
    }
    void prefill(Env& e, int P, int Tn, int n_draft = 0) {
        std::vector<Seg> segs{Seg{&e, P, Tn, 0, n_draft}};
        prefill_rows(segs, Tn);
    }

    GemvArgs gemv_args(const void* W, int ldw, const void* xin, const void* norm_w, const void* bias, const void* res, void* y, int N, int K,
                       int epi) {
        GemvArgs a; a.W = W; a.ldw = ldw; a.x = xin; a.norm_w = norm_w; a.eps = c.rms_eps; a.bias = bias; a.res = res; a.y = y; a.N = N; a.K = K;
        a.epi = epi; a.part_val = part_val; a.part_idx = part_idx; a.w8 = nullptr; a.scale = nullptr; a.skip = nullptr; return a;
// ... 2736 lines not shown
        a.part_val = part_val_b; a.part_idx = part_idx_b;
        launch_gemv_mx4b(st, a);
        if (a.epi == EPI_ARGMAX) {
            launch_argmax_final_batched(st, part_val_b, part_idx_b, gemv_mx4b_grid(a.N, EPI_ARGMAX), a.B, d_tok_b);
            HIP_CHECK(hipMemcpyAsync(h_tok_b, d_tok_b, a.B * sizeof(int), hipMemcpyDeviceToHost, st));
            sync();
            if (host_tokens) for (int b = 0; b < a.B; ++b) host_tokens[b] = h_tok_b[b];
        }
        sync();
        LAUNCH_CHECK("op_gemv_mxfp4_batched");
    }
    void op_quant_fp8(const void* w, int64_t rows, int cols, void* w8, float* scale) override {
        REQUIRE(sizeof(T) == 2, "fp8 quantisation reads bf16 weights");
        REQUIRE(w && w8 && scale, "null pointer");
        REQUIRE(rows >= 0 && rows <= INT32_MAX && cols > 0 && cols % 16 == 0, "rows must be >= 0 and cols a positive multiple of 16");
        if (rows > 0) launch_quant_fp8_rows(st, w, cols, w8, scale, rows, cols);
        sync();
        LAUNCH_CHECK("op_quant_fp8");
    }
    void op_quant_mxfp4(const void* w, int64_t rows, int cols, void* q4, uint8_t* e8) override {
        REQUIRE(sizeof(T) == 2, "MXFP4 quantisation reads bf16 weights");
        REQUIRE(w && q4 && e8, "null pointer");
        REQUIRE(rows >= 0 && cols > 0 && cols % 32 == 0, "cols must be a positive multiple of 32");
        if (rows > 0) launch_quant_mxfp4_rows(st, w, cols, q4, e8, rows, cols);
        sync();
        LAUNCH_CHECK("op_quant_mxfp4");
    }
    void require_row_width(int n) {
        constexpr int EPC = Elt<T>::PER_CHUNK;
        REQUIRE(n > 0 && n % EPC == 0,
                std::string("n must be a positive multiple of the 16-byte chunk (") + std::to_string(EPC) + " values of the engine type)");
    }
    struct OpInts {
        int* d = nullptr;
        OpInts(const int32_t* host, size_t count) {
            HIP_CHECK(hipMalloc((void**)&d, (count ? count : 1) * sizeof(int)));
            if (count && hipMemcpy(d, host, count * sizeof(int), hipMemcpyHostToDevice) != hipSuccess) {
                (void)hipFree(d);
                REQUIRE(false, "op: list upload failed");
            }
        }
        ~OpInts() { (void)hipFree(d); }
        OpInts(const OpInts&) = delete;
        OpInts& operator=(const OpInts&) = delete;
    };
    void op_rmsnorm(const void* xi, const void* g, void* y, int rows, int n, float eps) override {
        REQUIRE(xi && g && y, "null pointer");
        REQUIRE(rows >= 0, "rows must be >= 0");
        require_row_width(n);
        launch_rmsnorm<T>(st, xi, g, y, rows, n, eps);
        sync();
        LAUNCH_CHECK("op_rmsnorm");
    }
    void op_layernorm(const void* xi, const void* g, const void* b, void* y, int rows, int n, float eps) override {
        REQUIRE(xi && g && b && y, "null pointer");
        REQUIRE(rows >= 0, "rows must be >= 0");
        require_row_width(n);
        launch_layernorm<T>(st, xi, g, b, y, rows, n, eps);
        sync();
        LAUNCH_CHECK("op_layernorm");
    }
    void op_rmsnorm_tap(const void* xi, const void* g, void* y, int rows, int n, float eps, int skip_value, void* y2, int y2_row_value,
                        int y2_cap) override {
        REQUIRE(xi && g && y && y2, "null pointer");
        REQUIRE(rows >= 0, "rows must be >= 0");
        require_row_width(n);
        REQUIRE(y2_cap >= 1 && y2_row_value >= 0, "y2_cap must be >= 1 and y2_row >= 0");
        const int32_t words[2] = {skip_value, y2_row_value};
        OpInts d(words, 2);
        launch_rmsnorm<T>(st, xi, g, y, rows, n, eps, d.d, y2, d.d + 1, y2_cap);
        sync();
        LAUNCH_CHECK("op_rmsnorm_tap");
    }
    void op_rmsnorm_indexed(const void* xi, int x_rows, const void* g, void* y, const int32_t* src_rows, const int32_t* tap_rows, void* tap,
                            int tap_cap, int rows, int n, float eps) override {
        REQUIRE(xi && g && y && src_rows && tap_rows && tap, "null pointer");
        REQUIRE(rows >= 0 && x_rows >= 1 && tap_cap >= 1, "rows must be >= 0, x_rows and tap_cap >= 1");
        require_row_width(n);
        for (int r = 0; r < rows; ++r) {
            REQUIRE(src_rows[r] >= 0 && src_rows[r] < x_rows, "src_rows entry out of range");
            REQUIRE(tap_rows[r] >= -1 && tap_rows[r] < tap_cap, "tap_rows entry out of range");
        }
        std::vector<int32_t> both(src_rows, src_rows + rows);
        both.insert(both.end(), tap_rows, tap_rows + rows);
        OpInts d(both.data(), both.size());
        launch_rmsnorm_indexed<T>(st, xi, g, y, d.d, d.d + rows, tap, rows, n, eps);
        sync();
        LAUNCH_CHECK("op_rmsnorm_indexed");
    }
    void op_gather_rows(const int32_t* src, int rows, const void* emb, int embed_rows, const void* ft, int feat_rows, void* out, int n,
                        int skip_value) override {
        REQUIRE(src && emb && ft && out, "null pointer");
        REQUIRE(rows >= 0 && embed_rows >= 1 && feat_rows >= 1, "rows must be >= 0, embed_rows and feat_rows >= 1");
        require_row_width(n);
        for (int r = 0; r < rows; ++r) REQUIRE(src[r] < embed_rows && src[r] >= -feat_rows, "src entry out of range");
        std::vector<int32_t> h(src, src + rows);
        h.push_back(skip_value);
        OpInts d(h.data(), h.size());
        launch_gather_rows<T>(st, d.d, emb, ft, out, rows, n, d.d + rows);
        sync();
        LAUNCH_CHECK("op_gather_rows");
    }
    void op_gather_rows_ragged(const int32_t* list, int rows, const void* emb, int embed_rows, void* out, int out_rows, int n) override {
        REQUIRE(list && emb && out, "null pointer");
        REQUIRE(rows >= 0 && embed_rows >= 1 && out_rows >= 1, "rows must be >= 0, embed_rows and out_rows >= 1");
        require_row_width(n);
// ... 185 lines not shown
        hdr_out[0] = ho.n;
        for (int r = 0; r < BEAM_MAX_W; ++r) {
            hdr_out[1 + r] = ho.len[r]; hdr_out[1 + BEAM_MAX_W + r] = ho.fin[r]; hdr_out[1 + 2 * BEAM_MAX_W + r] = ho.set_of[r]; score_out[r] = ho.score[r];
        }
        HIP_CHECK(hipMemcpy(ids_out, bm_ids[1], rows * sizeof(int), hipMemcpyDeviceToHost));
        HIP_CHECK(hipMemcpy(lps_out, bm_lps[1], rows * sizeof(float), hipMemcpyDeviceToHost));
        HIP_CHECK(hipMemcpy(tok_b, bm_tok, (size_t)B * sizeof(int), hipMemcpyDeviceToHost));
        if (n_cp) {
            HIP_CHECK(hipMemcpy(pair_src, bm_pair_src, (size_t)BEAM_MAX_W * n_cp * sizeof(int), hipMemcpyDeviceToHost));
            HIP_CHECK(hipMemcpy(pair_dst, bm_pair_dst, (size_t)BEAM_MAX_W * n_cp * sizeof(int), hipMemcpyDeviceToHost));
        }
        HIP_CHECK(hipMemcpy(rec, bm_rec, BEAM_REC * sizeof(int), hipMemcpyDeviceToHost));
    }
    void kv_read(const LLayer& L, int env, int start, int n, float* k_out, float* v_out) {
        REQUIRE(k_out && v_out, "null output pointer");
        const int limit = env < 0 ? pages_total * PAGE : env_at(env).n_pages * PAGE;
        REQUIRE(start >= 0 && n >= 0 && start + n <= limit, "op_kv_read: positions outside the env's pages");
        const size_t page_elems = (size_t)nkv * PAGE * 128;
        std::vector<T> kp(page_elems), vp(page_elems);
        sync();
        for (int pg = start / PAGE; pg * PAGE < start + n; ++pg) {
            const int phys = env < 0 ? pg : envs[env].pages[pg];
            HIP_CHECK(hipMemcpy(kp.data(), L.kpool + (size_t)phys * page_elems, page_elems * sizeof(T), hipMemcpyDeviceToHost));
            HIP_CHECK(hipMemcpy(vp.data(), L.vpool + (size_t)phys * page_elems, page_elems * sizeof(T), hipMemcpyDeviceToHost));
            for (int off = 0; off < PAGE; ++off) {
                const int p = pg * PAGE + off;
                if (p < start || p >= start + n) continue;
                for (int kh = 0; kh < nkv; ++kh)
                    for (int d = 0; d < 128; ++d) {
                        const size_t o = ((size_t)(p - start) * nkv + kh) * 128 + d;
                        k_out[o] = host_to_f32(kp[((size_t)kh * PAGE + off) * 128 + d]);
                        v_out[o] = host_to_f32(vp[((size_t)kh * 128 + d) * PAGE + off]);
                    }
            }
        }
    }
    void op_llm_qkv_rope(const void* xin, int Tn, int P, void* q_out, int q_stride, int32_t* fused) override {
        REQUIRE(xin && q_out && fused, "null pointer");
        REQUIRE(Tn >= 1 && P >= 0 && P + Tn <= c.max_positions, "positions out of range");
        REQUIRE(q_stride >= nq * 128, "q_stride");
        Env& e = env_at(0);
        op_env_begin(0, P + Tn);
        const LLayer& L = ll[0];
        HIP_CHECK(hipMemcpyAsync(xn, xin, (size_t)Tn * H * sizeof(T), hipMemcpyDeviceToDevice, st));
        const Seg g{&e, P, Tn, 0};
        const bool roped = prefill_qkv(L, Tn, &g);
        if (!roped) prefill_rope_append(L, g);
        HIP_CHECK(hipMemcpy2DAsync(q_out, (size_t)q_stride * sizeof(T), qkv, (size_t)qkv_dim * sizeof(T), (size_t)nq * 128 * sizeof(T), Tn,
                                   hipMemcpyDeviceToDevice, st));
        sync();
        LAUNCH_CHECK("op_llm_qkv_rope");
        *fused = roped ? 1 : 0;
    }
    void op_rope_append(Env& e, const LLayer& L, void* rows, int ld, int Tn, int P) {
        RopeKvArgs r; r.Kpool = L.kpool; r.Vpool = L.vpool; r.page_table = e.d_pages; r.rope_tab = rope_tab; r.nq = nq; r.nkv = nkv; r.dyn_pos = nullptr;
        r.ld = ld; r.qkv = rows; r.T = Tn; r.P = P;
        launch_rope_kv<T>(st, r);
    }
    void op_attention_llm(void* qkv_new, int ld, int Tn, int P, const void* ctx, int ctx_T, void* out, int o_stride, int nsplit) override {
        Env& e = env_at(0);
        REQUIRE(ctx_T == P, "context length must equal P");
        op_env_begin(0, P + Tn);
        const LLayer& L = ll[0];
        if (ctx_T > 0) op_rope_append(e, L, const_cast<void*>(ctx), ld, ctx_T, 0);
        op_rope_append(e, L, qkv_new, ld, Tn, P);
        AttnArgs a = llm_attn_args(L, e, qkv_new, ld, out, o_stride, Tn, P, P + Tn, false);
        if (nsplit > 1) {
            REQUIRE(Tn * (nq / nkv) <= 32, "split-KV path takes at most 32 rows per kv head");
            a.nsplit = nsplit_max; a.tiles_per_split = tiles_per_split; a.rows_pad = 32;
            launch_attention<T>(st, a, 128, 1);
            launch_attention_combine<T>(st, a, 128);
        } else {
            launch_attention<T>(st, a, 128, 4);
            if (a.nsplit > 1) launch_attention_combine<T>(st, a, 128);
        }
        sync();
    }
    void op_attention_decode(int B, const void* ctx, int ld, int64_t ctx_rows, const int32_t* pos, const void* qkv_new, void* out,
                             int o_stride) override {
        REQUIRE(B == 1 || B == 2 || B == 4 || B == 8, "B must be 1, 2, 4 or 8");
        REQUIRE(B <= c.max_envs, "B exceeds max_envs");
        REQUIRE(pos && qkv_new && out, "null pointer");
        REQUIRE(ld >= qkv_dim && o_stride >= nq * 128, "row strides");
        const LLayer& L = ll[0];
        const bool keep = B == 1 && !ctx && pos[0] > 0;
        for (int b = 0; b < B; ++b) {
            REQUIRE(pos[b] >= 0 && pos[b] < c.max_positions && (keep || pos[b] <= ctx_rows), "decode position out of range");
            REQUIRE(pos[b] == 0 || ctx || keep, "null context rows");
            if (!keep) reset_env(b);
        }
        if (keep) REQUIRE(pos[0] < env_at(0).n_pages * PAGE, "null context rows: env 0 holds no page for this position (run the op that fills it first)");
        for (int b = 0; b < B && !keep; ++b) {
            Env& e = env_at(b);
            op_env_begin(b, pos[b] + 1);
            if (pos[b] > 0) op_rope_append(e, L, (char*)const_cast<void*>(ctx) + (size_t)b * ctx_rows * ld * sizeof(T), ld, pos[b], 0);
        }
        HIP_CHECK(hipMemcpy2DAsync(qkv, (size_t)qkv_dim * sizeof(T), qkv_new, (size_t)ld * sizeof(T), (size_t)qkv_dim * sizeof(T), B,
                                   hipMemcpyDeviceToDevice, st));
        if (B == 1) {
            h_ctl->pos = pos[0]; h_ctl->kv_len = pos[0] + 1; h_ctl->done = 0; h_ctl->count = 0; h_ctl->max_new = 0; h_ctl->n_eos = 0;
            h_ctl->draw0 = h_ctl->stream = 0;
            HIP_CHECK(hipMemcpyAsync(d_ctl, h_ctl, sizeof(GenCtl), hipMemcpyHostToDevice, st));
            decode_attention(decode_attn_args(L, env_at(0)));
        } else {
            for (int b = 0; b < B; ++b) { h_slots[b].page_table = envs[b].d_pages; h_slots[b].pos = pos[b]; h_slots[b].pad = 0; }
            HIP_CHECK(hipMemcpyAsync(d_slots, h_slots, B * sizeof(DecodeSlot), hipMemcpyHostToDevice, st));
            decode_attention(batched_decode_attn_args(L, B));
        }
        HIP_CHECK(hipMemcpy2DAsync(out, (size_t)o_stride * sizeof(T), attn, (size_t)nq * 128 * sizeof(T), (size_t)nq * 128 * sizeof(T), B,
                                   hipMemcpyDeviceToDevice, st));
        sync();
        LAUNCH_CHECK("op_attention_decode");
    }
    void op_attention_verify(int rows, const void* ctx, int ld, int ctx_rows, const void* qkv_new, void* out, int o_stride) override {
        REQUIRE(rows >= 1 && rows <= MAXB && rows * (nq / nkv) <= 32, "rows must be 1 .. 8 with rows * (q_heads / kv_heads) <= 32");
        REQUIRE(qkv_new && out, "null pointer");
        REQUIRE(ld >= qkv_dim && o_stride >= nq * 128, "row strides");
        REQUIRE(ctx_rows >= 0 && ctx_rows + rows <= c.max_positions, "verify positions out of range");
        REQUIRE(ctx_rows == 0 || ctx, "null context rows");
        set_speculative_buffers();
        const LLayer& L = ll[0];
        Env& e = env_at(0);
        op_env_begin(0, ctx_rows + rows);
        if (ctx_rows > 0) op_rope_append(e, L, const_cast<void*>(ctx), ld, ctx_rows, 0);
        HIP_CHECK(hipMemcpy2DAsync(qkv, (size_t)qkv_dim * sizeof(T), qkv_new, (size_t)ld * sizeof(T), (size_t)qkv_dim * sizeof(T), rows,
                                   hipMemcpyDeviceToDevice, st));
        h_ctl->pos = ctx_rows; h_ctl->kv_len = ctx_rows + 1; h_ctl->done = 0; h_ctl->count = 0; h_ctl->max_new = 0; h_ctl->n_eos = 0;
        h_ctl->draw0 = h_ctl->stream = 0;
        HIP_CHECK(hipMemcpyAsync(d_ctl, h_ctl, sizeof(GenCtl), hipMemcpyHostToDevice, st));
// ... 667 lines not shown
    if (!q4 || !e8 || !x) throw std::runtime_error("null pointer");
    if (N < 1 || K < 32 || K % 32 != 0 || ldw % 32 != 0 || ldw < K) throw std::runtime_error("K and ldw must be multiples of 32, ldw >= K, N >= 1");
    if (epi != EPI_NONE && epi != EPI_SWIGLU && epi != EPI_ARGMAX) throw std::runtime_error("epilogue: EPI_NONE, EPI_SWIGLU or EPI_ARGMAX");
    if (epi == EPI_SWIGLU && N % 64 != 0) throw std::runtime_error("SwiGLU needs N % 64 == 0 (32-row gate / up blocks)");
    if (epi != EPI_ARGMAX && !y) throw std::runtime_error("null output pointer");
    GemvArgs a; a.W = nullptr; a.ldw = ldw; a.x = x; a.norm_w = norm_w; a.eps = eps; a.bias = bias; a.res = res; a.y = y; a.N = N; a.K = K; a.epi = epi;
    a.part_val = nullptr; a.part_idx = nullptr; a.w8 = nullptr; a.scale = nullptr; a.skip = nullptr; a.w4 = q4; a.e8 = (const uint8_t*)e8;
    h->impl->op_gemv(a, host_token);
    API_END
}
int svln_op_gemv_mxfp4_batched(svln_engine* h, const void* q4, const void* e8, int ldw, const void* x, int ldx, const void* bias, const void* res,
                               int ldr, void* y, int ldy, int N, int K, int epi, int B, int32_t* host_tokens) {
    API_BEGIN_H
    GemvMx4BatchArgs a; a.q4 = q4; a.e8 = (const uint8_t*)e8; a.ldw = ldw; a.x = x; a.ldx = ldx; a.bias = bias; a.res = res; a.ldr = ldr;
    a.y = y; a.ldy = ldy; a.N = N; a.K = K; a.epi = epi; a.B = B; a.part_val = nullptr; a.part_idx = nullptr;
    h->impl->op_gemv_mxfp4_batched(a, host_tokens);
    API_END
}
int svln_op_gemv_mxfp4_batched_argmax_pen(svln_engine* h, const void* q4, const void* e8, int ldw, const void* x, int ldx, int N, int K, int B,
                                          const void* pen_flags, const int32_t* pen_rows, float penalty, int32_t* host_tokens) {
    API_BEGIN_H
    if (!pen_flags || !pen_rows) throw std::runtime_error("null pointer");
    GemvMx4BatchArgs a; a.q4 = q4; a.e8 = (const uint8_t*)e8; a.ldw = ldw; a.x = x; a.ldx = ldx; a.bias = nullptr; a.res = nullptr; a.ldr = 0;
    a.y = nullptr; a.ldy = 0; a.N = N; a.K = K; a.epi = EPI_ARGMAX; a.B = B; a.part_val = nullptr; a.part_idx = nullptr;
    a.pen_flags = (const uint8_t*)pen_flags; a.pen_rows = pen_rows; a.pen = penalty;
    h->impl->op_gemv_mxfp4_batched(a, host_tokens);
    API_END
}
int svln_op_rmsnorm(svln_engine* h, const void* x, const void* g, void* y, int rows, int n, float eps) { API_BEGIN_H h->impl->op_rmsnorm(x, g, y, rows, n, eps); API_END }
int svln_op_layernorm(svln_engine* h, const void* x, const void* g, const void* b, void* y, int rows, int n, float eps) {
    API_BEGIN_H h->impl->op_layernorm(x, g, b, y, rows, n, eps); API_END
}
int svln_op_rmsnorm_tap(svln_engine* h, const void* x, const void* g, void* y, int rows, int n, float eps, int skip_value, void* y2, int y2_row_value,
                        int y2_cap) {
    API_BEGIN_H h->impl->op_rmsnorm_tap(x, g, y, rows, n, eps, skip_value, y2, y2_row_value, y2_cap); API_END
}
int svln_op_rmsnorm_indexed(svln_engine* h, const void* x, int x_rows, const void* g, void* y, const int32_t* src_rows, const int32_t* tap_rows,
                            void* tap, int tap_cap, int rows, int n, float eps) {
    API_BEGIN_H h->impl->op_rmsnorm_indexed(x, x_rows, g, y, src_rows, tap_rows, tap, tap_cap, rows, n, eps); API_END
}
int svln_op_gather_rows(svln_engine* h, const int32_t* src, int rows, const void* embed, int embed_rows, const void* feats, int feat_rows, void* out,
                        int n, int skip_value) {
    API_BEGIN_H h->impl->op_gather_rows(src, rows, embed, embed_rows, feats, feat_rows, out, n, skip_value); API_END
}
int svln_op_gather_rows_ragged(svln_engine* h, const int32_t* list, int rows, const void* embed, int embed_rows, void* out, int out_rows, int n) {
    API_BEGIN_H h->impl->op_gather_rows_ragged(list, rows, embed, embed_rows, out, out_rows, n); API_END
}
int svln_op_frame_hash(svln_engine* h, const void* pix_dev, int F, int64_t words_per_frame, uint64_t* out_keys) {
    API_BEGIN_H h->impl->op_frame_hash(pix_dev, F, words_per_frame, out_keys); API_END
}
int svln_op_attention_llm(svln_engine* h, void* qkv, int ld, int T, int P, const void* ctx, int ctx_T, void* out, int o_stride, int nsplit) {
    API_BEGIN_H h->impl->op_attention_llm(qkv, ld, T, P, ctx, ctx_T, out, o_stride, nsplit); API_END
}
int svln_op_attention_vit(svln_engine* h, const void* qkv, int ld, int F, void* out, int o_stride) { API_BEGIN_H h->impl->op_attention_vit(qkv, ld, F, out, o_stride); API_END }
int svln_op_attention_decode(svln_engine* h, int B, const void* ctx_qkv, int ld, int64_t ctx_rows, const int32_t* pos, const void* qkv_new, void* out,
                             int o_stride) {
    API_BEGIN_H h->impl->op_attention_decode(B, ctx_qkv, ld, ctx_rows, pos, qkv_new, out, o_stride); API_END
}
int svln_op_attention_verify(svln_engine* h, int rows, const void* ctx_qkv, int ld, int ctx_rows, const void* qkv_new, void* out, int o_stride) {
    API_BEGIN_H h->impl->op_attention_verify(rows, ctx_qkv, ld, ctx_rows, qkv_new, out, o_stride); API_END
}
int svln_op_attention_verify_multi(svln_engine* h, int n_seq, int rows_max, const void* ctx_qkv, int ld, int ctx_rows, const int32_t* ctx_len, const void* qkv_new, const int32_t* rows, int share, void* out, int o_stride) {
    API_BEGIN_H h->impl->op_attention_verify_multi(n_seq, rows_max, ctx_qkv, ld, ctx_rows, ctx_len, qkv_new, rows, share, out, o_stride); API_END
}
int svln_op_verify_step(svln_engine* h, int rows, const int32_t* fed, const int32_t* cand, int count, int max_new, const int64_t* eos, int n_eos,
                        int32_t* new_count, int32_t* done, int64_t* emitted, int32_t* next_token) {
    API_BEGIN_H h->impl->op_verify_step(rows, fed, cand, count, max_new, eos, n_eos, new_count, done, emitted, next_token); API_END
}
int svln_op_kv_read(svln_engine* h, int env, int start, int n, float* k_out, float* v_out) { API_BEGIN_H h->impl->op_kv_read(env, start, n, k_out, v_out); API_END }
int svln_op_llm_qkv_rope(svln_engine* h, const void* x, int T, int P, void* q_out, int q_stride, int32_t* fused) {
    API_BEGIN_H h->impl->op_llm_qkv_rope(x, T, P, q_out, q_stride, fused); API_END
}
int svln_op_set_pages(svln_engine* h, int env, const int32_t* pages, int n) { API_BEGIN_H h->impl->op_set_pages(env, pages, n); API_END }
int svln_op_fill_attn_state(svln_engine* h, float pool_value, int part_nan) { API_BEGIN_H h->impl->op_fill_attn_state(pool_value, part_nan); API_END }
int svln_op_vit_qkv_attention(svln_engine* h, int layer, const void* x, int F, void* qkv_out, void* attn_out, int o_stride, int force_split,
                              int32_t* packer) {
    API_BEGIN_H h->impl->op_vit_qkv_attention(layer, x, F, qkv_out, attn_out, o_stride, force_split, packer); API_END
}
int svln_op_fill_vit_state(svln_engine* h, float pool_value, int part_nan) { API_BEGIN_H h->impl->op_fill_vit_state(pool_value, part_nan); API_END }
int svln_op_vit_kv_read(svln_engine* h, float* k_out, float* v_out) { API_BEGIN_H h->impl->op_vit_kv_read(k_out, v_out); API_END }
int svln_op_pool(svln_engine* h, const void* in, void* out, int F) { API_BEGIN_H h->impl->op_pool(in, out, F); API_END }
int svln_op_patchify(svln_engine* h, const float* pix, void* out, int F) { API_BEGIN_H h->impl->op_patchify(pix, out, F); API_END }

}
```

streamvln_amd/csrc/kernels.h:

```cpp
#pragma once
#include <hip/hip_runtime.h>
#include <stdint.h>

#include <vector>

namespace svln {

enum Epi : int { EPI_NONE = 0, EPI_GELU_TANH = 1, EPI_GELU_ERF = 2, EPI_SWIGLU = 3, EPI_ARGMAX = 4, EPI_ARGMAX_LSE = 5, EPI_SAMPLE = 6, EPI_TARGET = 7,
                 EPI_ARGMAX_LSE_TOPK = 8, EPI_SAMPLE_TOPK = 9 };
constexpr int TOPK_C = 8;
constexpr bool epi_is_topk(int epi) { return epi == EPI_ARGMAX_LSE_TOPK || epi == EPI_SAMPLE_TOPK; }
constexpr bool epi_is_argmax(int epi) { return epi == EPI_ARGMAX || epi == EPI_ARGMAX_LSE || epi == EPI_SAMPLE || epi == EPI_TARGET || epi_is_topk(epi); }
struct TargetArgs { const int* tgt = nullptr; float* tgt_val = nullptr; float inv_t = 1.0f; };
struct SampleArgs {
    const int* stream = nullptr; const int* draw = nullptr; const int* count = nullptr;
    float inv_t = 1.0f; uint32_t seed_lo = 0, seed_hi = 0;
    float* part_raw = nullptr; float* part_max = nullptr;
};

struct RopeKvArgs;
struct VitPackArgs { void* Kpool; void* Vpool; int F, S, heads, head_dim; };
struct GemmArgs {
    const void* A; int lda;
    const void* W; int ldw;
// ... 107 lines not shown
                        const float* part_raw = nullptr, const float* part_max = nullptr);
struct GemvSubsetArgs {
    const int* ids = nullptr; int n = 0;
    const void* W = nullptr; int ldw = 0;
    const void* x = nullptr; int ldx = 0;
    int V = 0, K = 0, B = 0, epi = EPI_ARGMAX;
    float tg_inv_t = 1.0f;
    float* part_val = nullptr; int* part_idx = nullptr; float* part_sum = nullptr;
    const uint8_t* pen_flags = nullptr; const int* pen_rows = nullptr; float pen = 1.0f;
    SampleArgs smp;
    const int* skip = nullptr;
};
template <typename T> void launch_gemv_subset(hipStream_t s, const GemvSubsetArgs& a);
void launch_subset_logprobs(hipStream_t s, const float* src, int n, int B, float* out, const int* row_dev = nullptr, const int* skip = nullptr);
void launch_topk_merge(hipStream_t s, const float* cand_val, const int* cand_idx, int n_part, int c, int B, int k, const float* part_val,
                       const int* part_idx, const float* part_sum, const float* part_max, int* top_ids, float* top_logprobs,
                       const int* row_dev = nullptr, const int* skip = nullptr);
void launch_truncate_partials(hipStream_t s, const float* cand_val, const int* cand_idx, int n_part, int c, int B, int top_k, float top_p,
                              const SampleArgs& smp, float* tr_val, int* tr_idx, float* tr_sum, const int* skip = nullptr);
void launch_gumbel(hipStream_t s, uint32_t seed_lo, uint32_t seed_hi, int stream, int draw, int n0, int count, float* out);
void launch_verify_feed(hipStream_t s, const GenCtl* ctl, const int* token, const int* draft, int* vctl, int* fed, int rows, int max_positions);
template <typename T> void launch_verify_step(hipStream_t s, const int* fed, const int* cand, const int* n_rows, int max_rows, GenCtl* ctl,
                                              const int* eos, int* out_ids, int* out_token, const void* xn, void* hid_tap, int H, int tap_cap,
                                              int* stats);
void launch_set_flags(hipStream_t s, uint8_t* flags, const int* ids, const int* count, int n_host, int value);

struct DecodeSlot { const int* page_table; int pos; int pad; };

constexpr int ATTN_PART_PAD = 4;
struct AttnArgs {
    const void* Q; int q_stride;
    void* O; int o_stride;
    const void* Kpool; const void* Vpool;
    const int* page_table;
    int n_kv_total, hpf, G, T;
    int P;
    int kv_len;
    const int* dyn_kv_len;
    float scale;
    int causal;
    int nsplit, tiles_per_split;
    float* part;
    int rows_pad;
    int fuse_rope_append;
    const float* rope_tab;
    const int* dyn_pos;
    int nq_heads;
    const DecodeSlot* slots;
    size_t part_bstride;
    int batch;
    const int* skip;
    int key_groups;
    const int* dyn_rows;
};
template <typename T> void launch_attention(hipStream_t s, const AttnArgs& a, int head_dim, int waves);
template <typename T> void launch_attention_verify(hipStream_t s, const AttnArgs& a);
template <typename T> void launch_attention_verify_multi(hipStream_t s, const AttnArgs& a);
template <typename T> void launch_attention_combine(hipStream_t s, const AttnArgs& a, int head_dim);
template <typename T> int attn_key_groups(int head_dim);

struct DecodeLayerArgs {
    const float* part; int nsplit, tiles_per_split; const int* dyn_kv_len; int n_kv, Gq;
    const void *o_w, *post_norm, *gu_w, *down_w;
    const void *next_norm, *next_qkv_w, *next_qkv_b;
    void* x;
    void* qkv_out;
    int H, I, qd, qkv_dim; float eps;
    unsigned long long* gran[4];
    unsigned* seq;
    unsigned* giveup;
    const int* skip;
    unsigned long long* dbg;
};
template <typename T> bool decode_layer_supported(const DecodeLayerArgs& a, int cus);
template <typename T> void launch_decode_layer(hipStream_t s, const DecodeLayerArgs& a, int cus, hipEvent_t start = nullptr, hipEvent_t stop = nullptr);
void decode_layer_init_attrs();
struct DecodeLayerWalkOp { int elem_size, K, nrows, pair, first; };
struct DecodeLayerWalkSlot { int64_t load_off; int32_t valid, row, pb, row_done; };
int decode_layer_walk(const DecodeLayerWalkOp& op, const DecodeLayerWalkOp& next, int wave, int lane, DecodeLayerWalkSlot* out, int max_slots,
                      int64_t* refill);

template <typename T> void launch_rmsnorm(hipStream_t s, const void* x, const void* g, void* y, int rows, int n, float eps, const int* skip = nullptr,
                                          void* y2 = nullptr, const int* y2_row = nullptr, int y2_cap = 0);
template <typename T> void launch_rmsnorm_indexed(hipStream_t s, const void* x, const void* g, void* y, const int* src_rows, const int* tap_rows,
                                                  void* tap, int rows, int n, float eps);
template <typename T> void launch_layernorm(hipStream_t s, const void* x, const void* g, const void* b, void* y, int rows, int n, float eps);

struct RopeKvArgs {
    void* qkv; int ld;
    void* Kpool; void* Vpool;
    const int* page_table;
    const float* rope_tab;
    int T, nq, nkv, P;
    const int* dyn_pos;
};
template <typename T> void launch_rope_kv(hipStream_t s, const RopeKvArgs& a);
void launch_rope_table(hipStream_t s, float* tab, const float* inv_freq, int positions);
void launch_frame_hash(hipStream_t s, const float* pix, int F, size_t words_per_frame, unsigned long long* out);

template <typename T> void launch_vit_kv_pack(hipStream_t s, const void* qkv, int ld, void* Kpool, void* Vpool, int F, int S,
                                             int heads, int head_dim);

template <typename T> void launch_patchify(hipStream_t s, const float* pix, void* out, int F, int image, int patch, int kp);

template <typename T> void launch_pool(hipStream_t s, const void* in, void* out, const int* tap_idx, const float* tap_w, int F,
                                       int side, int out_side, int C);

template <typename T> void launch_memory_prune(hipStream_t s, const void* m, int n_rows, int H, int keep, float* partial, float* mean, float* score,
                                               int* sel);
template <typename T> void launch_gather_rows(hipStream_t s, const int* src, const void* embed, const void* feats, void* out,
                                              int rows, int n, const int* skip = nullptr);
template <typename T> void launch_gather_rows_ragged(hipStream_t s, const int* list, const void* embed, void* out, int rows, int n);

template <typename T> void launch_kv_page_copy(hipStream_t s, void* const* pools, int n_pools, int src_page, const int* dst_pages, int n_dst,
                                               int64_t page_elems);

template <typename T> void launch_kv_page_gather(hipStream_t s, void* const* pools, int n_pools, const int* src_pages, const int* dst_pages, int n,
                                                 int64_t page_elems);

constexpr int BEAM_MAX_W = 8, BEAM_CP_MAX = 8, BEAM_REC = 4 + 3 * BEAM_MAX_W;
struct BeamHdr { int n; int len[BEAM_MAX_W]; int fin[BEAM_MAX_W]; int set_of[BEAM_MAX_W]; float score[BEAM_MAX_W]; };
struct BeamSelectArgs {
    const int* list_ids = nullptr; const float* list_lps = nullptr;
    const BeamHdr* in = nullptr; const int* in_ids = nullptr; const float* in_lps = nullptr;
    BeamHdr* out = nullptr; int* out_ids = nullptr; float* out_lps = nullptr;
    int len_cap = 0, W = 0, limit = 0, n_eos = 0, B = 0, n_cp = 0, set_stride = 0;
    const int* eos = nullptr; const int* set_pages = nullptr;
    int *tok_b = nullptr, *pair_src = nullptr, *pair_dst = nullptr, *rec = nullptr;
};
void launch_beam_select(hipStream_t s, const BeamSelectArgs& a);

struct RowMap { int blk, nint, phase; };
template <typename T> void launch_synth(hipStream_t s, void* dst, int dst_ld, int64_t rows, int cols, RowMap m, uint64_t seed_t,
                                        float half_width, float base);
template <typename T> void launch_convert(hipStream_t s, void* dst, int dst_ld, int64_t rows, int cols, RowMap m, const void* src,
                                          int src_is_f32);
template <typename T> void launch_to_f32(hipStream_t s, const void* src, float* dst, int64_t n);
template <typename T> void launch_from_f32(hipStream_t s, const float* src, void* dst, int64_t n);

struct ResampleAxis { int ksize = 0; std::vector<int> xmin, cnt, k; };
struct ResampleDev { const int *hmin, *hcnt, *hk, *vmin, *vcnt, *vk; int ks_h, ks_v; };
void build_resample_table(int in_size, int out_size, ResampleAxis& ax);
void build_normalize_lut(float* lut256, float mean, float std);
size_t preprocess_lds_bytes(int W, int S, int ks_v, int ks_h);
void launch_preprocess(hipStream_t s, const uint8_t* rgb, float* out, int n_frames, int H, int W, int S, const ResampleDev& t, const float* lut);
void launch_upload(hipStream_t s, const void* src_dev_visible, void* dst, size_t bytes);
void preprocess_init_attrs();
// ... 22 lines not shown
```

streamvln_amd/csrc/misc.hip:

```cpp
#include <stdexcept>

#include "common.h"
#include "kernels.h"

namespace svln {

namespace {

template <typename T>
__device__ __forceinline__ void rmsnorm_row(const T* xr, const T* g, T* yr, T* y2r, int n, float eps, int lane) {
    constexpr int EPC = Elt<T>::PER_CHUNK;
    const int nch = n / EPC;
    float ss = 0.0f;
    for (int ci = lane; ci < nch; ci += 64) {
        float f[EPC];
        chunk_to_f32<T>(*(const uint4*)(xr + (size_t)ci * EPC), f);
#pragma unroll
        for (int e = 0; e < EPC; ++e) ss += f[e] * f[e];
    }
    ss = wave_sum(ss);
    const float sc = rsqrtf(ss / (float)n + eps);
    for (int ci = lane; ci < nch; ci += 64) {
        float f[EPC], gf[EPC];
        chunk_to_f32<T>(*(const uint4*)(xr + (size_t)ci * EPC), f);
        chunk_to_f32<T>(*(const uint4*)(g + (size_t)ci * EPC), gf);
#pragma unroll
        for (int e = 0; e < EPC; ++e) f[e] = gf[e] * (f[e] * sc);
        const uint4 o = f32_to_chunk<T>(f);
        *(uint4*)(yr + (size_t)ci * EPC) = o;
        if (y2r) *(uint4*)(y2r + (size_t)ci * EPC) = o;
    }
}
template <typename T>
__global__ __launch_bounds__(256) void rmsnorm_kernel(const T* x, const T* g, T* y, int rows, int n, float eps, const int* skip, T* y2,
                                                      const int* y2_row, int y2_cap) {
    if (skip && *skip) return;
    const int lane = threadIdx.x & 63;
    const int row = blockIdx.x * 4 + (threadIdx.x >> 6);
    if (row >= rows) return;
    T* y2r = y2 ? y2 + (size_t)min(*y2_row + row, y2_cap - 1) * n : nullptr;
    rmsnorm_row<T>(x + (size_t)row * n, g, y + (size_t)row * n, y2r, n, eps, lane);
}
template <typename T>
__global__ __launch_bounds__(256) void rmsnorm_indexed_kernel(const T* x, const T* g, T* y, const int* src_rows, const int* tap_rows, T* tap,
                                                              int rows, int n, float eps) {
    const int lane = threadIdx.x & 63;
    const int row = blockIdx.x * 4 + (threadIdx.x >> 6);
    if (row >= rows) return;
    const int t = tap_rows[row];
    rmsnorm_row<T>(x + (size_t)src_rows[row] * n, g, y + (size_t)row * n, t >= 0 ? tap + (size_t)t * n : nullptr, n, eps, lane);
}

template <typename T>
__global__ __launch_bounds__(256) void layernorm_kernel(const T* x, const T* g, const T* b, T* y, int rows, int n, float eps) {
    constexpr int EPC = Elt<T>::PER_CHUNK;
    const int lane = threadIdx.x & 63;
    const int row = blockIdx.x * 4 + (threadIdx.x >> 6);
    if (row >= rows) return;
    const T* xr = x + (size_t)row * n;
    T* yr = y + (size_t)row * n;
    const int nch = n / EPC;
    float s = 0.0f;
    for (int ci = lane; ci < nch; ci += 64) {
        float f[EPC];
        chunk_to_f32<T>(*(const uint4*)(xr + (size_t)ci * EPC), f);
#pragma unroll
        for (int e = 0; e < EPC; ++e) s += f[e];
    }
    const float mu = wave_sum(s) / (float)n;
    float v = 0.0f;
    for (int ci = lane; ci < nch; ci += 64) {
        float f[EPC];
        chunk_to_f32<T>(*(const uint4*)(xr + (size_t)ci * EPC), f);
#pragma unroll
        for (int e = 0; e < EPC; ++e) v += (f[e] - mu) * (f[e] - mu);
    }
    const float sc = rsqrtf(wave_sum(v) / (float)n + eps);
    for (int ci = lane; ci < nch; ci += 64) {
        float f[EPC], gf[EPC], bf[EPC];
        chunk_to_f32<T>(*(const uint4*)(xr + (size_t)ci * EPC), f);
        chunk_to_f32<T>(*(const uint4*)(g + (size_t)ci * EPC), gf);
        chunk_to_f32<T>(*(const uint4*)(b + (size_t)ci * EPC), bf);
#pragma unroll
        for (int e = 0; e < EPC; ++e) f[e] = (f[e] - mu) * sc * gf[e] + bf[e];
        *(uint4*)(yr + (size_t)ci * EPC) = f32_to_chunk<T>(f);
    }
}

template <typename T>
__global__ __launch_bounds__(256) void rope_kv_kernel(RopeKvArgs p) {
    const int i = blockIdx.x, hd = blockIdx.y * 4 + (threadIdx.x >> 6), d = threadIdx.x & 63;
    if (hd >= p.nq + 2 * p.nkv) return;
    const int P = p.dyn_pos ? *p.dyn_pos : p.P;
    const int pos = P + i;
    T* row = (T*)p.qkv + (size_t)i * p.ld + (size_t)hd * 128;
    const float x1 = to_f32(row[d]), x2 = to_f32(row[d + 64]);
    const int page = p.page_table[pos >> 6], off = pos & 63;
    if (hd < p.nq + p.nkv) {
        const float c = p.rope_tab[(size_t)pos * 128 + d], s = p.rope_tab[(size_t)pos * 128 + 64 + d];
        const float o1 = x1 * c - x2 * s, o2 = x2 * c + x1 * s;
        if (hd < p.nq) {
            row[d] = from_f32<T>(o1);
            row[d + 64] = from_f32<T>(o2);
        } else {
            const int kh = hd - p.nq;
            T* kr = (T*)p.Kpool + (((size_t)page * p.nkv + kh) * 64 + off) * 128;
            kr[d] = from_f32<T>(o1);
            kr[d + 64] = from_f32<T>(o2);
        }
    } else {
        const int kh = hd - p.nq - p.nkv;
        T* vt = (T*)p.Vpool + ((size_t)page * p.nkv + kh) * 128 * 64;
        vt[(size_t)d * 64 + off] = from_f32<T>(x1);
        vt[(size_t)(d + 64) * 64 + off] = from_f32<T>(x2);
    }
}

__global__ __launch_bounds__(64) void rope_table_kernel(float* tab, const float* inv_freq, int positions) {
    const int pos = blockIdx.x, d = threadIdx.x;
    const float ang = (float)pos * inv_freq[d];
    tab[(size_t)pos * 128 + d] = cosf(ang);
    tab[(size_t)pos * 128 + 64 + d] = sinf(ang);
}

__global__ __launch_bounds__(256) void frame_hash_kernel(const uint32_t* pix, size_t words_per_frame, unsigned long long* out) {
    const int f = blockIdx.y;
    const uint32_t* p = pix + (size_t)f * words_per_frame;
    unsigned long long a = 0, b = 0;
    for (size_t i = (size_t)blockIdx.x * 256 + threadIdx.x; i < words_per_frame; i += (size_t)gridDim.x * 256) {
        const uint64_t v = (uint64_t)p[i] | ((uint64_t)i << 32);
        a += splitmix64(v ^ 0x243F6A8885A308D3ull);
        b += splitmix64(v * 0x9E3779B97F4A7C15ull + 0x13198A2E03707344ull);
    }
    atomicAdd(out + 2 * f, a);
    atomicAdd(out + 2 * f + 1, b);
}

template <typename T>
__global__ __launch_bounds__(256) void vit_kv_pack_kernel(const T* qkv, int ld, T* Kpool, T* Vpool, int F, int S, int heads, int HD,
                                                          int HDP, int VROWS) {
    extern __shared__ __attribute__((aligned(16))) char pack_smem[];
    constexpr int EPC = Elt<T>::PER_CHUNK;
    T* vt = (T*)pack_smem;
    const int tile = blockIdx.x, kh = blockIdx.y;
    const int f = kh / heads, head = kh % heads, Hv = heads * HD;
    const int nkv = F * heads;
    const int hc = HD / EPC, hpc = HDP / EPC, pitch = HD + EPC;
    T* kp = Kpool + ((size_t)tile * nkv + kh) * 64 * HDP;
    T* vp = Vpool + ((size_t)tile * nkv + kh) * VROWS * 64;
    const uint4 zero = make_uint4(0, 0, 0, 0);
    for (int e = threadIdx.x; e < 64 * hpc; e += 256) {
        const int key = e / hpc, cchunk = e % hpc, s = tile * 64 + key;
        uint4 v = zero;
        if (s < S && cchunk < hc) v = *(const uint4*)(qkv + (size_t)(f * S + s) * ld + Hv + head * HD + cchunk * EPC);
        *(uint4*)(kp + (size_t)key * HDP + cchunk * EPC) = v;
    }
    for (int e = threadIdx.x; e < 64 * hc; e += 256) {
        const int key = e / hc, cchunk = e % hc, s = tile * 64 + key;
        uint4 v = zero;
        if (s < S) v = *(const uint4*)(qkv + (size_t)(f * S + s) * ld + 2 * Hv + head * HD + cchunk * EPC);
        *(uint4*)(vt + key * pitch + cchunk * EPC) = v;
    }
    __syncthreads();
    constexpr int KC = 64 / EPC;
    for (int e = threadIdx.x; e < VROWS * KC; e += 256) {
        const int d = e / KC, kc = e % KC;
        T out[EPC];
// ... 179 lines not shown
        const unsigned long long b = __ballot(f != 0);
        const int before = __popcll(b & ((1ull << lane) - 1ull));
        if (lane == 0) wtot[wave] = __popcll(b);
        __syncthreads();
        int off = base;
        for (int w = 0; w < wave; ++w) off += wtot[w];
        if (f) sel[off + before] = i;
        __syncthreads();
        if (tid == 0) { int t = 0; for (int w = 0; w < 16; ++w) t += wtot[w]; base += t; }
        __syncthreads();
    }
}

SVLN_DEV int64_t map_row(int64_t r, RowMap m) { return (r / m.blk) * (int64_t)m.blk * m.nint + (int64_t)m.phase * m.blk + r % m.blk; }

template <typename T>
__global__ __launch_bounds__(256) void synth_kernel(T* dst, int dst_ld, int64_t rows, int cols, RowMap m, uint64_t seed_t, float step,
                                                    float base) {
    const int64_t total = rows * cols;
    for (int64_t i = (int64_t)blockIdx.x * 256 + threadIdx.x; i < total; i += (int64_t)gridDim.x * 256) {
        const int64_t r = i / cols;
        const int c = (int)(i - r * cols);
        dst[map_row(r, m) * dst_ld + c] = from_f32<T>(to_f32((bf16)synth_value(seed_t, (uint64_t)i, step, base)));
    }
}

template <typename T>
__global__ __launch_bounds__(256) void convert_kernel(T* dst, int dst_ld, int64_t rows, int cols, RowMap m, const void* src, int src_is_f32) {
    const int64_t total = rows * cols;
    for (int64_t i = (int64_t)blockIdx.x * 256 + threadIdx.x; i < total; i += (int64_t)gridDim.x * 256) {
        const int64_t r = i / cols;
        const int c = (int)(i - r * cols);
        const float v = src_is_f32 ? ((const float*)src)[i] : to_f32(((const bf16*)src)[i]);
        dst[map_row(r, m) * dst_ld + c] = from_f32<T>(v);
    }
}

template <typename T> __global__ void to_f32_kernel(const T* s, float* d, int64_t n) {
    for (int64_t i = (int64_t)blockIdx.x * 256 + threadIdx.x; i < n; i += (int64_t)gridDim.x * 256) d[i] = to_f32(s[i]);
}
template <typename T> __global__ void from_f32_kernel(const float* s, T* d, int64_t n) {
    for (int64_t i = (int64_t)blockIdx.x * 256 + threadIdx.x; i < n; i += (int64_t)gridDim.x * 256) d[i] = from_f32<T>(s[i]);
}

int grid_for(int64_t n) {
    int64_t g = (n + 255) / 256;
    return (int)(g < 1 ? 1 : (g > 8192 ? 8192 : g));
}

}



template <typename T> void launch_rmsnorm(hipStream_t s, const void* x, const void* g, void* y, int rows, int n, float eps, const int* skip,
                                          void* y2, const int* y2_row, int y2_cap) {
    if (rows <= 0) return;
    hipLaunchKernelGGL((rmsnorm_kernel<T>), dim3((rows + 3) / 4), dim3(256), 0, s, (const T*)x, (const T*)g, (T*)y, rows, n, eps, skip, (T*)y2,
                       y2_row, y2_cap);
}
template <typename T> void launch_rmsnorm_indexed(hipStream_t s, const void* x, const void* g, void* y, const int* src_rows, const int* tap_rows,
                                                  void* tap, int rows, int n, float eps) {
    if (rows <= 0) return;
    hipLaunchKernelGGL((rmsnorm_indexed_kernel<T>), dim3((rows + 3) / 4), dim3(256), 0, s, (const T*)x, (const T*)g, (T*)y, src_rows, tap_rows,
                       (T*)tap, rows, n, eps);
}
template <typename T> void launch_layernorm(hipStream_t s, const void* x, const void* g, const void* b, void* y, int rows, int n, float eps) {
    if (rows <= 0) return;
    hipLaunchKernelGGL((layernorm_kernel<T>), dim3((rows + 3) / 4), dim3(256), 0, s, (const T*)x, (const T*)g, (const T*)b, (T*)y, rows, n, eps);
}
template <typename T> void launch_rope_kv(hipStream_t s, const RopeKvArgs& a) {
    hipLaunchKernelGGL((rope_kv_kernel<T>), dim3(a.T, (a.nq + 2 * a.nkv + 3) / 4), dim3(256), 0, s, a);
}
void launch_frame_hash(hipStream_t s, const float* pix, int F, size_t words_per_frame, unsigned long long* out) {
    hipLaunchKernelGGL(frame_hash_kernel, dim3(64, F), dim3(256), 0, s, (const uint32_t*)pix, words_per_frame, out);
}
void launch_rope_table(hipStream_t s, float* tab, const float* inv_freq, int positions) {
    hipLaunchKernelGGL(rope_table_kernel, dim3(positions), dim3(64), 0, s, tab, inv_freq, positions);
}
template <typename T> void launch_vit_kv_pack(hipStream_t s, const void* qkv, int ld, void* Kpool, void* Vpool, int F, int S, int heads,
                                             int head_dim) {
    constexpr int EPC = Elt<T>::PER_CHUNK;
    const int hdc = (((head_dim + EPC - 1) / EPC) + 1) & ~1;
    const int vrows = ((head_dim + 31) / 32) * 32;
    const size_t lds = (size_t)64 * (head_dim + EPC) * sizeof(T);
    hipLaunchKernelGGL((vit_kv_pack_kernel<T>), dim3((S + 63) / 64, F * heads), dim3(256), lds, s, (const T*)qkv, ld, (T*)Kpool, (T*)Vpool, F, S,
                       heads, head_dim, hdc * EPC, vrows);
}
template <typename T> void launch_patchify(hipStream_t s, const float* pix, void* out, int F, int image, int patch, int kp) {
    const int side = image / patch;
    hipLaunchKernelGGL((patchify_kernel<T>), dim3(F * side * side), dim3(256), 0, s, pix, (T*)out, F, image, patch, kp);
}
template <typename T> void launch_pool(hipStream_t s, const void* in, void* out, const int* tap_idx, const float* tap_w, int F, int side,
                                       int out_side, int C) {
    hipLaunchKernelGGL((pool_kernel<T>), dim3(F * out_side * out_side), dim3(256), 0, s, (const T*)in, (T*)out, tap_idx, tap_w, side, out_side, C);
}
template <typename T> void launch_gather_rows(hipStream_t s, const int* src, const void* embed, const void* feats, void* out, int rows, int n,
                                              const int* skip) {
    if (rows <= 0) return;
    hipLaunchKernelGGL((gather_rows_kernel<T>), dim3(rows), dim3(256), 0, s, src, (const T*)embed, (const T*)feats, (T*)out, n, skip);
}
template <typename T> void launch_gather_rows_ragged(hipStream_t s, const int* list, const void* embed, void* out, int rows, int n) {
    if (rows <= 0) return;
    hipLaunchKernelGGL((gather_rows_ragged_kernel<T>), dim3(rows), dim3(256), 0, s, (const int2*)list, (const T*)embed, (T*)out, n);
}
void launch_verify_feed(hipStream_t s, const GenCtl* ctl, const int* token, const int* draft, int* vctl, int* fed, int rows, int max_positions) {
    hipLaunchKernelGGL(verify_feed_kernel, dim3(1), dim3(64), 0, s, ctl, token, draft, vctl, fed, rows, max_positions);
}
template <typename T> void launch_verify_step(hipStream_t s, const int* fed, const int* cand, const int* n_rows, int max_rows, GenCtl* ctl,
                                              const int* eos, int* out_ids, int* out_token, const void* xn, void* hid_tap, int H, int tap_cap,
                                              int* stats) {
    hipLaunchKernelGGL((verify_step_kernel<T>), dim3(1), dim3(256), 0, s, fed, cand, n_rows, max_rows, ctl, eos, out_ids, out_token, (const T*)xn,
                       (T*)hid_tap, H, tap_cap, stats);
}
template <typename T> void launch_memory_prune(hipStream_t s, const void* m, int n_rows, int H, int keep, float* partial, float* mean, float* score,
                                               int* sel) {
    const int nb = (n_rows + 63) / 64;
    hipLaunchKernelGGL((mem_colsum_kernel<T>), dim3((H + 255) / 256, nb), dim3(256), 0, s, (const T*)m, n_rows, H, partial);
    hipLaunchKernelGGL(mem_mean_kernel, dim3((H + 255) / 256), dim3(256), 0, s, partial, nb, n_rows, H, mean);
    hipLaunchKernelGGL((mem_score_kernel<T>), dim3((n_rows + 3) / 4), dim3(256), 0, s, (const T*)m, n_rows, H, mean, score);
    int* flag = (int*)partial;
    hipLaunchKernelGGL(mem_rank_kernel, dim3((n_rows + 3) / 4), dim3(256), 0, s, score, n_rows, keep, flag);
    hipLaunchKernelGGL(mem_compact_kernel, dim3(1), dim3(1024), 0, s, flag, n_rows, sel);
}
// ... 215 lines not shown
            for (int k = 0; k < len; ++k) { oi[k] = ii[k]; ol[k] = il[k]; }
            int nlen = len;
            if (!a.in->fin[pr]) {
                const int tok = a.list_ids[pr * a.W + pj];
                oi[len] = tok; ol[len] = a.list_lps[pr * a.W + pj];
                nlen = len + 1;
                fin = nlen >= a.limit;
                for (int k = 0; k < a.n_eos; ++k) fin |= a.eos[k] == tok;
            }
            a.out->len[tid] = nlen; a.out->fin[tid] = fin; a.out->score[tid] = s_score[it];
        }
        s_live[tid] = !fin;
    }
    __syncthreads();
    int first = -1, n_live = 0;
    for (int c = BEAM_MAX_W - 1; c >= 0; --c) if (s_live[c]) { first = c; ++n_live; }
    if (tid < a.B && first >= 0) {
        const int c = tid < n_new && s_live[tid] ? tid : first;
        a.tok_b[tid] = a.out_ids[(size_t)c * a.len_cap + a.out->len[c] - 1];
    }
    if (tid == 0) {
        unsigned held = 0, claimed = 0;
        int n_rows = 0, np = 0;
        for (int q = 0; q < n; ++q) { held |= 1u << a.in->set_of[q]; n_rows += a.in->fin[q] ? 0 : 1; }
        for (int c = 0; c < BEAM_MAX_W; ++c) {
            if (c >= n_new) { a.rec[4 + c] = -1; a.rec[4 + BEAM_MAX_W + c] = -1; a.rec[4 + 2 * BEAM_MAX_W + c] = -1; continue; }
            const int it = s_sel[c], src = a.in->set_of[it >> 3];
            int dst = src;
            if ((claimed >> src) & 1u) {
                dst = __ffs((int)(~(held | claimed) & 0xFFFFu)) - 1;
                for (int i = 0; i < a.n_cp; ++i) {
                    a.pair_src[np] = a.set_pages[src * a.set_stride + i];
                    a.pair_dst[np] = a.set_pages[dst * a.set_stride + i];
                    ++np;
                }
            }
            claimed |= 1u << dst;
            a.out->set_of[c] = dst;
            a.rec[4 + c] = it >> 3; a.rec[4 + BEAM_MAX_W + c] = it & 7; a.rec[4 + 2 * BEAM_MAX_W + c] = dst;
        }
        a.out->n = n_new;
        a.rec[0] = n_new; a.rec[1] = n_live; a.rec[2] = n_rows; a.rec[3] = np;
    }
}
}
void launch_beam_select(hipStream_t s, const BeamSelectArgs& a) {
    if (a.W < 1 || a.W > BEAM_MAX_W || a.B < 1 || a.B > 64 || a.limit < 1 || a.limit > a.len_cap || a.n_cp < 0 || a.n_cp > BEAM_CP_MAX || a.n_eos < 0)
        throw std::runtime_error("beam select: W must be 1 .. 8, limit 1 .. len_cap, n_cp 0 .. 8");
    hipLaunchKernelGGL(beam_select_kernel, dim3(1), dim3(64), 0, s, a);
}

#define SVLN_INST(T)                                                                                                              \
    template void launch_rmsnorm<T>(hipStream_t, const void*, const void*, void*, int, int, float, const int*, void*, const int*, int);                              \
    template void launch_rmsnorm_indexed<T>(hipStream_t, const void*, const void*, void*, const int*, const int*, void*, int, int, float);                          \
    template void launch_layernorm<T>(hipStream_t, const void*, const void*, const void*, void*, int, int, float);               \
    template void launch_gather_rows_ragged<T>(hipStream_t, const int*, const void*, void*, int, int);                            \
    template void launch_rope_kv<T>(hipStream_t, const RopeKvArgs&);                                                              \
    template void launch_vit_kv_pack<T>(hipStream_t, const void*, int, void*, void*, int, int, int, int);                         \
    template void launch_patchify<T>(hipStream_t, const float*, void*, int, int, int, int);                                       \
    template void launch_pool<T>(hipStream_t, const void*, void*, const int*, const float*, int, int, int, int);                  \
    template void launch_gather_rows<T>(hipStream_t, const int*, const void*, const void*, void*, int, int, const int*);                      \
    template void launch_verify_step<T>(hipStream_t, const int*, const int*, const int*, int, GenCtl*, const int*, int*, int*, const void*,    \
                                        void*, int, int, int*);                                                                  \
    template void launch_memory_prune<T>(hipStream_t, const void*, int, int, int, float*, float*, float*, int*);                   \
    template void launch_synth<T>(hipStream_t, void*, int, int64_t, int, RowMap, uint64_t, float, float);                          \
    template void launch_convert<T>(hipStream_t, void*, int, int64_t, int, RowMap, const void*, int);                              \
    template void launch_to_f32<T>(hipStream_t, const void*, float*, int64_t);                                                    \
    template void launch_from_f32<T>(hipStream_t, const float*, void*, int64_t);
SVLN_INST(bf16)
SVLN_INST(float)

}
```

Before: 182.0.

## Balance causal prefill attention, tile rope/KV scatter, add register-resident rmsnorm

Adds a load-balanced causal prefill attention launch. A host-built workgroup table splits the long tail blocks into two key-range halves and sorts all work by length, with a combine pass over only the split rows. It also adds a page-tiled rope/KV-scatter kernel that writes V transposed through LDS with vector stores, and an rmsnorm variant that keeps the row in registers, both picked by default for large row counts. These aim to cut causal load imbalance and uncoalesced scatter and norm traffic. In exchange they add host-side plan caching with events, a combine launch, and new code paths.

```diff
diff --git a/include/streamvln_hip.h b/include/streamvln_hip.h
--- a/include/streamvln_hip.h
+++ b/include/streamvln_hip.h
@@ -240,6 +240,7 @@
                           const int32_t* draws, int32_t* host_tokens, float* host_logprobs, float* host_y, float* host_dist);
 int svln_op_rmsnorm(svln_engine* h, const void* x, const void* g, void* y, int rows, int n, float eps);
 int svln_op_layernorm(svln_engine* h, const void* x, const void* g, const void* b, void* y, int rows, int n, float eps);
+int svln_op_norm_rows(svln_engine* h, const void* x, const void* g, void* y, int rows, int n, float eps, int form);
 int svln_op_rmsnorm_tap(svln_engine* h, const void* x, const void* g, void* y, int rows, int n, float eps, int skip_value, void* y2, int y2_row_value,
                         int y2_cap);
 int svln_op_rmsnorm_indexed(svln_engine* h, const void* x, int x_rows, const void* g, void* y, const int32_t* src_rows, const int32_t* tap_rows,
@@ -250,7 +251,10 @@
 int svln_op_frame_hash(svln_engine* h, const void* pix_dev, int F, int64_t words_per_frame, uint64_t* out_keys);
 int svln_op_attention_llm(svln_engine* h, void* qkv, int ld, int T, int P, const void* ctx_qkv, int ctx_T, void* out, int o_stride,
                           int nsplit);
+int svln_op_attention_balanced(svln_engine* h, void* qkv, int ld, int T, int P, const void* ctx_qkv, int ctx_T, void* out, int o_stride,
+                               int thr, int32_t* info);
 int svln_op_attention_vit(svln_engine* h, const void* qkv, int ld, int F, void* out, int o_stride);
+int svln_op_rope_kv(svln_engine* h, void* qkv, int ld, int T, int P, int form);
 int svln_op_attention_decode(svln_engine* h, int B, const void* ctx_qkv, int ld, int64_t ctx_rows, const int32_t* pos, const void* qkv_new,
                              void* out, int o_stride);
 int svln_op_attention_verify(svln_engine* h, int rows, const void* ctx_qkv, int ld, int ctx_rows, const void* qkv_new, void* out,
diff --git a/streamvln_amd/_lib.py b/streamvln_amd/_lib.py
--- a/streamvln_amd/_lib.py
+++ b/streamvln_amd/_lib.py
@@ -216,6 +216,7 @@
     "svln_op_gumbel": (_I, [_P, _U64, _I, _I, _I, _I, _PF]),
     "svln_op_subset_argmax": (_I, [_P, _P, _I, _P, _I, _I, _I, _I, _PI64, _I, _P, _P, _F, _F, _U64, _PI32, _PI32, _PI32, _PF, _PF, _PF]),
     "svln_op_rmsnorm": (_I, [_P, _P, _P, _P, _I, _I, _F]),
+    "svln_op_norm_rows": (_I, [_P, _P, _P, _P, _I, _I, _F, _I]),
     "svln_op_layernorm": (_I, [_P, _P, _P, _P, _P, _I, _I, _F]),
     "svln_op_rmsnorm_tap": (_I, [_P, _P, _P, _P, _I, _I, _F, _I, _P, _I, _I]),
     "svln_op_rmsnorm_indexed": (_I, [_P, _P, _I, _P, _P, _PI32, _PI32, _P, _I, _I, _I, _F]),
@@ -223,6 +224,8 @@
     "svln_op_gather_rows_ragged": (_I, [_P, _PI32, _I, _P, _I, _P, _I, _I]),
     "svln_op_frame_hash": (_I, [_P, _P, _I, _I64, C.POINTER(C.c_uint64)]),
     "svln_op_attention_llm": (_I, [_P, _P, _I, _I, _I, _P, _I, _P, _I, _I]),
+    "svln_op_rope_kv": (_I, [_P, _P, _I, _I, _I, _I]),
+    "svln_op_attention_balanced": (_I, [_P, _P, _I, _I, _I, _P, _I, _P, _I, _I, _P]),
     "svln_op_attention_vit": (_I, [_P, _P, _I, _I, _P, _I]),
     "svln_op_attention_decode": (_I, [_P, _I, _P, _I, _I64, _PI32, _P, _P, _I]),
     "svln_op_attention_verify": (_I, [_P, _I, _P, _I, _I, _P, _P, _I]),
diff --git a/streamvln_amd/csrc/attention.hip b/streamvln_amd/csrc/attention.hip
--- a/streamvln_amd/csrc/attention.hip
+++ b/streamvln_amd/csrc/attention.hip
@@ -1,4 +1,6 @@
+#include <algorithm>
 #include <type_traits>
+#include <vector>
 
 #include "common.h"
 #include "kernels.h"
@@ -34,9 +36,16 @@
     if constexpr (I < N) { f(std::integral_constant<int, I>{}); static_for<I + 1, N>(f); }
 }
 
-template <typename T, int HD, int WAVES, int KG = 1, int PF = 1>
+template <typename T, int HD, int WAVES, int KG = 1, int PF = 1, bool BAL = false>
 __global__ __launch_bounds__(WAVES * 64 * KG, (KG == 1 && WAVES == 4 && sizeof(T) == 2) ? 2 : 1) void attn_kernel(AttnArgs p) {
     using G = AttnGeom<T, HD>;
+    static_assert(!BAL || KG == 1, "the balanced launch has no key groups");
+    int4 ent = make_int4(0, 0, 0, 0);
+    if constexpr (BAL) ent = p.wg_table[blockIdx.x];
+    const int bx = BAL ? ent.x : (int)blockIdx.x;
+    const int zslot = BAL ? (ent.y >> 16) - 1 : (p.nsplit > 1 ? (int)blockIdx.z : -1);
+    const int zbase = BAL ? ent.z : (int)blockIdx.z * p.tiles_per_split;
+    const int zend = BAL ? ent.w : zbase + p.tiles_per_split;
     constexpr int NT = WAVES * 64;
     constexpr int EPC = G::EPC;
     extern __shared__ __attribute__((aligned(16))) char smem[];
@@ -46,14 +55,14 @@
 
     const int tid = KG == 1 ? (int)threadIdx.x : (int)threadIdx.x - kg * NT, lane = tid & 63, wave = tid >> 6;
     const int r = lane & 31, h = lane >> 5;
-    const int kh = blockIdx.y;
+    const int kh = BAL ? (ent.y & 0xffff) : (int)blockIdx.y;
     const int frame = kh / p.hpf, head0 = (kh % p.hpf) * p.G;
-    const int kt0 = blockIdx.z * p.tiles_per_split + kg;
+    const int kt0 = zbase + kg;
     const int page0 = p.page_table ? p.page_table[kt0] : kt0;
     const int kv_len = p.dyn_kv_len ? *p.dyn_kv_len : p.kv_len;
     const int P = p.dyn_kv_len ? kv_len - p.T : p.P;
     const int rows_total = p.T * p.G;
-    const int rho = (blockIdx.x * WAVES + wave) * 32 + r;
+    const int rho = (bx * WAVES + wave) * 32 + r;
     const bool valid = rho < rows_total;
     const int qi = valid ? rho / p.G : 0;
     const int qg = valid ? rho - qi * p.G : 0;
@@ -70,13 +79,13 @@
     }
     int tiles = (kv_len + 63) >> 6;
     if (p.causal) {
-        const int last_row = min((int)(blockIdx.x + 1) * WAVES * 32, rows_total) - 1;
+        const int last_row = min((bx + 1) * WAVES * 32, rows_total) - 1;
         const int last_pos = P + last_row / p.G;
         tiles = min(tiles, (last_pos >> 6) + 1);
     }
-    const int kt_begin = blockIdx.z * p.tiles_per_split + kg;
-    const int kt_end = min(tiles, (int)blockIdx.z * p.tiles_per_split + p.tiles_per_split);
-    const int n_iter = (kt_end - (int)blockIdx.z * p.tiles_per_split + KG - 1) / KG;
+    const int kt_begin = zbase + kg;
+    const int kt_end = min(tiles, zend);
+    const int n_iter = (kt_end - zbase + KG - 1) / KG;
 
     const float scale2 = p.scale * 1.4426950408889634f;
     f32x16 O[G::DT];
@@ -201,7 +210,7 @@
         }
 
         const int tile_last_key = kt * 64 + 63;
-        const bool need_mask = tile_last_key >= kv_len || (p.causal && tile_last_key > P + (int)(blockIdx.x * WAVES * 32) / p.G);
+        const bool need_mask = tile_last_key >= kv_len || (p.causal && tile_last_key > P + (bx * WAVES * 32) / p.G);
         if (need_mask) {
 #pragma unroll
             for (int j = 0; j < 2; ++j)
@@ -316,7 +325,7 @@
         __syncthreads();
         for (int q = threadIdx.x; q < ROWS * (HD / 4); q += NT * KG) {
             const int row = q / (HD / 4), c4 = q - row * (HD / 4);
-            const int rho_o = blockIdx.x * ROWS + row;
+            const int rho_o = bx * ROWS + row;
             if (rho_o >= rows_total) continue;
             float4 acc = *(const float4*)(sO + (size_t)row * OP + c4 * 4);
 #pragma unroll
@@ -341,8 +350,8 @@
     }
     if (!valid) return;
 
-    if (p.nsplit > 1) {
-        float* dst = p.part + (((size_t)blockIdx.z * p.n_kv_total + kh) * p.rows_pad + rho) * (HD + ATTN_PART_PAD);
+    if (zslot >= 0) {
+        float* dst = p.part + (((size_t)zslot * p.n_kv_total + kh) * p.rows_pad + (rho - p.part_row0)) * (HD + ATTN_PART_PAD);
 #pragma unroll
         for (int d = 0; d < G::DT; ++d)
 #pragma unroll
@@ -753,7 +762,7 @@
     if (p.skip && *p.skip) return;
     const int wave = threadIdx.x >> 6, lane = threadIdx.x & 63;
     float* wsh = wsh_all[wave];
-    const int rho = blockIdx.x * (blockDim.x >> 6) + wave, kh = blockIdx.y, env = blockIdx.z;
+    const int rho = p.part_row0 + blockIdx.x * (blockDim.x >> 6) + wave, kh = blockIdx.y, env = blockIdx.z;
     int kv_len;
     if constexpr (VERIFY && MULTI) {
         const int rows = min(p.slots[env].pad, p.T);
@@ -770,7 +779,7 @@
     const int tiles = (kv_len + 63) >> 6;
     const int nsplit = min(min(p.nsplit, 64), (tiles + p.tiles_per_split - 1) / p.tiles_per_split);
     const size_t split_stride = (size_t)p.n_kv_total * p.rows_pad * (HD + ATTN_PART_PAD);
-    const float* base = p.part + (size_t)env * p.part_bstride + ((size_t)kh * p.rows_pad + rho) * (HD + ATTN_PART_PAD);
+    const float* base = p.part + (size_t)env * p.part_bstride + ((size_t)kh * p.rows_pad + (rho - p.part_row0)) * (HD + ATTN_PART_PAD);
     float mz = -INFINITY, lz = 0.0f;
     if (lane < nsplit) { mz = base[lane * split_stride + HD]; lz = base[lane * split_stride + HD + 1]; }
     const float mstar = wave_max(mz);
@@ -836,8 +845,47 @@
         if (waves == 1) launch_attn_t<T, 72, 1>(s, a); else launch_attn_t<T, 72, 4>(s, a);
     }
 }
+bool attn_balance_plan(int T, int P, int G, int n_kv, int& thr, std::vector<int>& table, int* row0, int* rows_pad) {
+    const int rows = T * G, blocks = (rows + 127) / 128;
+    std::vector<int> cnt(blocks);
+    long sum = 0;
+    for (int b = 0; b < blocks; ++b) {
+        const int last_row = std::min((b + 1) * 128, rows) - 1;
+        cnt[b] = ((P + last_row / G) >> 6) + 1;
+        sum += cnt[b];
+    }
+    if (thr < 0) thr = (int)((sum + blocks - 1) / blocks);
+    int first = blocks;
+    while (first > 0 && cnt[first - 1] > thr) --first;
+    table.clear();
+    if (first == blocks) return false;
+    struct Ent { int len, v[4]; };
+    std::vector<Ent> es;
+    es.reserve((size_t)(2 * blocks - first) * n_kv);
+    for (int b = 0; b < blocks; ++b)
+        for (int kh = 0; kh < n_kv; ++kh) {
+            if (b < first) { es.push_back({cnt[b], {b, kh, 0, cnt[b]}}); continue; }
+            const int h = (cnt[b] + 1) / 2;
+            es.push_back({h, {b, kh | (1 << 16), 0, h}});
+            if (cnt[b] > h) es.push_back({cnt[b] - h, {b, kh | (2 << 16), h, cnt[b]}});
+            else es.push_back({0, {b, kh | (2 << 16), 0, 0}});
+        }
+    std::stable_sort(es.begin(), es.end(), [](const Ent& x, const Ent& y) { return x.len > y.len; });
+    table.reserve(es.size() * 4);
+    for (const Ent& e : es) table.insert(table.end(), e.v, e.v + 4);
+    *row0 = first * 128;
+    *rows_pad = (blocks - first) * 128;
+    return true;
+}
+template <typename T> void launch_attention_balanced(hipStream_t s, const AttnArgs& a) {
+    using G = AttnGeom<T, 128>;
+    if (!(a.wg_table && a.n_wgs > 0 && a.causal && a.key_groups <= 1 && a.nsplit == 2 && a.part && a.part_row0 >= 0 && a.part_row0 % 128 == 0 &&
+          a.part_row0 + a.rows_pad >= a.T * a.G))
+        throw std::runtime_error("balanced attention: a causal launch with a workgroup table, two partial slots and the cut rows inside rows_pad");
+    hipLaunchKernelGGL((attn_kernel<T, 128, 4, 1, 1, true>), dim3(a.n_wgs), dim3(256), G::K_TILE_BYTES + G::V_TILE_BYTES, s, a);
+}
 template <typename T> void launch_attention_combine(hipStream_t s, const AttnArgs& a, int head_dim) {
-    const int rows = a.T * a.G, rpw = rows >= 256 ? 4 : 1;
+    const int rows = a.T * a.G - a.part_row0, rpw = rows >= 256 ? 4 : 1;
     dim3 grid((rows + rpw - 1) / rpw, a.n_kv_total, a.batch > 0 ? a.batch : 1), block(64 * rpw);
     if (head_dim == 128) hipLaunchKernelGGL((attn_combine_kernel<T, 128>), grid, block, 0, s, a);
     else if (head_dim == 72) hipLaunchKernelGGL((attn_combine_kernel<T, 72>), grid, block, 0, s, a);
@@ -867,6 +915,8 @@
     set_max_lds((const void*)attn_verify_multi_kernel<float>, AttnGeom<float, 128>::K_TILE_BYTES + AttnGeom<float, 128>::V_TILE_BYTES);
     attn_attr<bf16, 128, 1>(); attn_attr<bf16, 128, 4>(); attn_attr<bf16, 72, 1>(); attn_attr<bf16, 72, 4>();
     attn_attr<float, 128, 1>(); attn_attr<float, 128, 4>(); attn_attr<float, 72, 1>(); attn_attr<float, 72, 4>();
+    set_max_lds((const void*)attn_kernel<bf16, 128, 4, 1, 1, true>, AttnGeom<bf16, 128>::K_TILE_BYTES + AttnGeom<bf16, 128>::V_TILE_BYTES);
+    set_max_lds((const void*)attn_kernel<float, 128, 4, 1, 1, true>, AttnGeom<float, 128>::K_TILE_BYTES + AttnGeom<float, 128>::V_TILE_BYTES);
     set_max_lds((const void*)attn_kernel<bf16, 72, 2, VitGroups<bf16>::KG, VitGroups<bf16>::PF>, GroupGeom<bf16, 72, VitGroups<bf16>::KG>::LDS);
     set_max_lds((const void*)attn_kernel<float, 72, 2, VitGroups<float>::KG, VitGroups<float>::PF>, GroupGeom<float, 72, VitGroups<float>::KG>::LDS);
 }
@@ -874,6 +924,8 @@
 template int attn_key_groups<bf16>(int);
 template int attn_key_groups<float>(int);
 template void launch_attention<bf16>(hipStream_t, const AttnArgs&, int, int);
+template void launch_attention_balanced<bf16>(hipStream_t, const AttnArgs&);
+template void launch_attention_balanced<float>(hipStream_t, const AttnArgs&);
 template void launch_attention<float>(hipStream_t, const AttnArgs&, int, int);
 template void launch_attention_verify<bf16>(hipStream_t, const AttnArgs&);
 template void launch_attention_verify<float>(hipStream_t, const AttnArgs&);
diff --git a/streamvln_amd/csrc/engine.hip b/streamvln_amd/csrc/engine.hip
--- a/streamvln_amd/csrc/engine.hip
+++ b/streamvln_amd/csrc/engine.hip
@@ -200,6 +200,9 @@
     virtual void op_gather_rows_ragged(const int32_t* list, int rows, const void* embed, int embed_rows, void* out, int out_rows, int n) = 0;
     virtual void op_frame_hash(const void* pix, int F, int64_t words_per_frame, uint64_t* out_keys) = 0;
     virtual void op_attention_llm(void* qkv, int ld, int T, int P, const void* ctx, int ctx_T, void* out, int o_stride, int nsplit) = 0;
+    virtual void op_rope_kv(void* rows, int ld, int T, int P, int form) = 0;
+    virtual void op_norm_rows(const void* x, const void* g, void* y, int rows, int n, float eps, int form) = 0;
+    virtual void op_attention_balanced(void* qkv, int ld, int T, int P, const void* ctx, int ctx_T, void* out, int o_stride, int thr, int32_t* info) = 0;
     virtual void op_attention_vit(const void* qkv, int ld, int F, void* out, int o_stride) = 0;
     virtual void op_attention_decode(int B, const void* ctx, int ld, int64_t ctx_rows, const int32_t* pos, const void* qkv_new, void* out,
                                      int o_stride) = 0;
@@ -252,6 +255,9 @@
     float* gemm_ws = nullptr; size_t gemm_ws_elems = 0; void* zero_line = nullptr;
     float* inv_freq; float* rope_tab;
     float* attn_part; size_t attn_part_elems = 0; int nsplit_max, tiles_per_split;
+    struct BalPlan { int Tn = -1, P = -1, thr = 0, n_wgs = 0, row0 = 0, rows_pad = 0; int4* d_table = nullptr; int* h_table = nullptr; hipEvent_t ev = nullptr; bool pending = false; };
+    static constexpr int BAL_PLANS = 4;
+    BalPlan bal_plans[BAL_PLANS]; int bal_next = 0; size_t bal_cap = 0; std::vector<int> bal_tmp;
     float* part_val; int* part_idx; int* d_token; float* d_top2;
     GenCtl* d_ctl;
     GenCtl* h_ctl = nullptr;
@@ -533,7 +539,16 @@
             constexpr int PW = 128 + ATTN_PART_PAD;
             const size_t dec = (size_t)MAXB * nsplit_max * nkv * 32 * PW, pre = (size_t)8 * nkv * PREFILL_SPLIT_ROWS * PW;
             attn_part_elems = dec > pre ? dec : pre;
+            const int bal_blocks = (c.max_positions * (nq / nkv) + 127) / 128;
+            const size_t bal = (size_t)2 * nkv * (bal_blocks / 2 + 1) * 128 * PW;
+            if (bal > attn_part_elems) attn_part_elems = bal;
             attn_part = dalloc<float>(attn_part_elems);
+            bal_cap = (size_t)2 * bal_blocks * nkv;
+            for (BalPlan& b : bal_plans) {
+                b.d_table = dalloc<int4>(bal_cap);
+                HIP_CHECK(hipHostMalloc((void**)&b.h_table, bal_cap * sizeof(int4)));
+                HIP_CHECK(hipEventCreateWithFlags(&b.ev, hipEventDisableTiming));
+            }
         }
         part_val = dalloc<float>(2048); part_idx = dalloc<int>(2048); part_sum = dalloc<float>(2048);
         d_scores = dalloc<float>((size_t)c.max_positions + 8, true); d_score_b = dalloc<float>(HEAD_ROWS + MAXB, true);
@@ -590,6 +605,10 @@
         }
         for (auto& pr : pp_ring) { if (pr.a) (void)hipEventDestroy(pr.a); if (pr.b) (void)hipEventDestroy(pr.b); }
         if (src_ev) (void)hipEventDestroy(src_ev);
+        for (BalPlan& b : bal_plans) {
+            if (b.h_table) (void)hipHostFree(b.h_table);
+            if (b.ev) (void)hipEventDestroy(b.ev);
+        }
         for (auto ev : ring_ev) (void)hipEventDestroy(ev);
         if (ring_host) (void)hipHostFree(ring_host);
         for (auto e : probe_ev) (void)hipEventDestroy(e);
@@ -1093,6 +1112,38 @@
         return a;
     }
 
+    void balance_prefill_attn(AttnArgs& a, int thr) {
+        if (!a.causal || a.nsplit != 1) return;
+        const int rows = a.T * a.G, wgs = ((rows + 127) / 128) * nkv, tiles = (a.kv_len + PAGE - 1) / PAGE;
+        if (thr < 0 && !(wgs >= 128 && tiles >= 4)) return;
+        BalPlan* bp = nullptr;
+        for (BalPlan& b : bal_plans) if (b.Tn == a.T && b.P == a.P && b.thr == thr) bp = &b;
+        if (!bp) {
+            bp = &bal_plans[bal_next]; bal_next = (bal_next + 1) % BAL_PLANS;
+            if (bp->pending) { HIP_CHECK(hipEventSynchronize(bp->ev)); bp->pending = false; }
+            bp->Tn = a.T; bp->P = a.P; bp->thr = thr; bp->n_wgs = 0;
+            int t = thr;
+            while (attn_balance_plan(a.T, a.P, a.G, nkv, t, bal_tmp, &bp->row0, &bp->rows_pad)) {
+                if ((size_t)2 * nkv * bp->rows_pad * (128 + ATTN_PART_PAD) <= attn_part_elems && bal_tmp.size() / 4 <= bal_cap) {
+                    bp->n_wgs = (int)(bal_tmp.size() / 4);
+                    std::memcpy(bp->h_table, bal_tmp.data(), bal_tmp.size() * sizeof(int));
+                    HIP_CHECK(hipMemcpyAsync(bp->d_table, bp->h_table, bal_tmp.size() * sizeof(int), hipMemcpyHostToDevice, st));
+                    HIP_CHECK(hipEventRecord(bp->ev, st));
+                    bp->pending = true;
+                    break;
+                }
+                ++t;
+            }
+        }
+        if (bp->n_wgs == 0) return;
+        a.wg_table = bp->d_table; a.n_wgs = bp->n_wgs; a.part_row0 = bp->row0; a.rows_pad = bp->rows_pad;
+        a.nsplit = 2; a.tiles_per_split = (tiles + 1) / 2;
+    }
+    void launch_prefill_attention(const AttnArgs& a) {
+        if (a.wg_table) launch_attention_balanced<T>(st, a); else launch_attention<T>(st, a, 128, 4);
+        if (a.nsplit > 1) launch_attention_combine<T>(st, a, 128);
+    }
+
     struct Seg { Env* e; int P, Tn, off; int n_draft = 0; };
     RopeKvArgs rope_kv_args(const LLayer& L, const Seg& g) {
         RopeKvArgs r; r.qkv = qkv + (size_t)g.off * qkv_dim; r.ld = qkv_dim; r.Kpool = L.kpool; r.Vpool = L.vpool; r.rope_tab = rope_tab;
@@ -1128,8 +1179,8 @@
                 T* q_g = qkv + (size_t)g.off * qkv_dim;
                 if (!roped) prefill_rope_append(L, g);
                 AttnArgs a = llm_attn_args(L, *g.e, q_g, qkv_dim, attn + (size_t)g.off * qd, qd, g.Tn, g.P, g.P + g.Tn, false);
-                launch_attention<T>(st, a, 128, 4);
-                if (a.nsplit > 1) launch_attention_combine<T>(st, a, 128);
+                balance_prefill_attn(a, -1);
+                launch_prefill_attention(a);
             }
             GemmArgs ao = gemm_args(attn, qd, L.o_w, qd, x, H, nullptr, x, H, 0, M, H, qd, EPI_NONE);
             ao.norm_w = L.post_norm; ao.norm_out = xn; ao.norm_eps = c.rms_eps;
@@ -3972,6 +4023,15 @@
         sync();
         LAUNCH_CHECK("op_rmsnorm");
     }
+    void op_norm_rows(const void* xi, const void* g, void* y, int rows, int n, float eps, int form) override {
+        REQUIRE(xi && g && y, "null pointer");
+        REQUIRE(rows >= 0, "rows must be >= 0");
+        REQUIRE(form >= 0 && form <= 2, "form");
+        require_row_width(n);
+        launch_rmsnorm_form<T>(st, xi, g, y, rows, n, eps, form);
+        sync();
+        LAUNCH_CHECK("op_norm_rows");
+    }
     void op_layernorm(const void* xi, const void* g, const void* b, void* y, int rows, int n, float eps) override {
         REQUIRE(xi && g && b && y, "null pointer");
         REQUIRE(rows >= 0, "rows must be >= 0");
@@ -4263,10 +4323,20 @@
         LAUNCH_CHECK("op_llm_qkv_rope");
         *fused = roped ? 1 : 0;
     }
-    void op_rope_append(Env& e, const LLayer& L, void* rows, int ld, int Tn, int P) {
+    void op_rope_append(Env& e, const LLayer& L, void* rows, int ld, int Tn, int P, int form = 0) {
         RopeKvArgs r; r.Kpool = L.kpool; r.Vpool = L.vpool; r.page_table = e.d_pages; r.rope_tab = rope_tab; r.nq = nq; r.nkv = nkv; r.dyn_pos = nullptr;
-        r.ld = ld; r.qkv = rows; r.T = Tn; r.P = P;
+        r.ld = ld; r.qkv = rows; r.T = Tn; r.P = P; r.form = form;
         launch_rope_kv<T>(st, r);
+    }
+    void op_rope_kv(void* rows, int ld, int Tn, int P, int form) override {
+        REQUIRE(rows, "null pointer");
+        REQUIRE(Tn >= 1 && P >= 0 && P + Tn <= c.max_positions, "positions out of range");
+        REQUIRE(ld >= qkv_dim, "row stride");
+        REQUIRE(form >= 0 && form <= 2, "form");
+        op_env_begin(0, P + Tn);
+        op_rope_append(env_at(0), ll[0], rows, ld, Tn, P, form);
+        sync();
+        LAUNCH_CHECK("op_rope_kv");
     }
     void op_attention_llm(void* qkv_new, int ld, int Tn, int P, const void* ctx, int ctx_T, void* out, int o_stride, int nsplit) override {
         Env& e = env_at(0);
@@ -4282,10 +4352,29 @@
             launch_attention<T>(st, a, 128, 1);
             launch_attention_combine<T>(st, a, 128);
         } else {
-            launch_attention<T>(st, a, 128, 4);
-            if (a.nsplit > 1) launch_attention_combine<T>(st, a, 128);
+            balance_prefill_attn(a, -1);
+            launch_prefill_attention(a);
         }
         sync();
+    }
+    void op_attention_balanced(void* qkv_new, int ld, int Tn, int P, const void* ctx, int ctx_T, void* out, int o_stride, int thr, int32_t* info) override {
+        REQUIRE(qkv_new && out && info, "null pointer");
+        REQUIRE(Tn >= 1 && P >= 0 && P + Tn <= c.max_positions, "positions out of range");
+        REQUIRE(ctx_T == P && (P == 0 || ctx), "context length must equal P");
+        REQUIRE(ld >= qkv_dim && o_stride >= nq * 128, "row strides");
+        REQUIRE(thr >= -2, "thr");
+        Env& e = env_at(0);
+        op_env_begin(0, P + Tn);
+        const LLayer& L = ll[0];
+        if (ctx_T > 0) op_rope_append(e, L, const_cast<void*>(ctx), ld, ctx_T, 0);
+        op_rope_append(e, L, qkv_new, ld, Tn, P);
+        AttnArgs a = llm_attn_args(L, e, qkv_new, ld, out, o_stride, Tn, P, P + Tn, false);
+        if (thr != -1) { a.nsplit = 1; a.tiles_per_split = pages_per_env; a.rows_pad = 32; }
+        if (thr >= -1) balance_prefill_attn(a, thr);
+        launch_prefill_attention(a);
+        sync();
+        LAUNCH_CHECK("op_attention_balanced");
+        info[0] = a.wg_table ? a.n_wgs : 0; info[1] = a.wg_table ? a.part_row0 : 0;
     }
     void op_attention_decode(int B, const void* ctx, int ld, int64_t ctx_rows, const int32_t* pos, const void* qkv_new, void* out,
                              int o_stride) override {
@@ -5059,6 +5148,16 @@
 int svln_op_attention_llm(svln_engine* h, void* qkv, int ld, int T, int P, const void* ctx, int ctx_T, void* out, int o_stride, int nsplit) {
     API_BEGIN_H h->impl->op_attention_llm(qkv, ld, T, P, ctx, ctx_T, out, o_stride, nsplit); API_END
 }
+int svln_op_norm_rows(svln_engine* h, const void* x, const void* g, void* y, int rows, int n, float eps, int form) {
+    API_BEGIN_H h->impl->op_norm_rows(x, g, y, rows, n, eps, form); API_END
+}
+int svln_op_rope_kv(svln_engine* h, void* qkv, int ld, int T, int P, int form) {
+    API_BEGIN_H h->impl->op_rope_kv(qkv, ld, T, P, form); API_END
+}
+int svln_op_attention_balanced(svln_engine* h, void* qkv, int ld, int T, int P, const void* ctx, int ctx_T, void* out, int o_stride, int thr,
+                               int32_t* info) {
+    API_BEGIN_H h->impl->op_attention_balanced(qkv, ld, T, P, ctx, ctx_T, out, o_stride, thr, info); API_END
+}
 int svln_op_attention_vit(svln_engine* h, const void* qkv, int ld, int F, void* out, int o_stride) { API_BEGIN_H h->impl->op_attention_vit(qkv, ld, F, out, o_stride); API_END }
 int svln_op_attention_decode(svln_engine* h, int B, const void* ctx_qkv, int ld, int64_t ctx_rows, const int32_t* pos, const void* qkv_new, void* out,
                              int o_stride) {
diff --git a/streamvln_amd/csrc/kernels.h b/streamvln_amd/csrc/kernels.h
--- a/streamvln_amd/csrc/kernels.h
+++ b/streamvln_amd/csrc/kernels.h
@@ -183,11 +183,15 @@
     const int* skip;
     int key_groups;
     const int* dyn_rows;
+    const int4* wg_table; int n_wgs;
+    int part_row0;
 };
 template <typename T> void launch_attention(hipStream_t s, const AttnArgs& a, int head_dim, int waves);
 template <typename T> void launch_attention_verify(hipStream_t s, const AttnArgs& a);
 template <typename T> void launch_attention_verify_multi(hipStream_t s, const AttnArgs& a);
 template <typename T> void launch_attention_combine(hipStream_t s, const AttnArgs& a, int head_dim);
+bool attn_balance_plan(int T, int P, int G, int n_kv, int& thr, std::vector<int>& table, int* row0, int* rows_pad);
+template <typename T> void launch_attention_balanced(hipStream_t s, const AttnArgs& a);
 template <typename T> int attn_key_groups(int head_dim);
 
 struct DecodeLayerArgs {
@@ -213,6 +217,7 @@
 
 template <typename T> void launch_rmsnorm(hipStream_t s, const void* x, const void* g, void* y, int rows, int n, float eps, const int* skip = nullptr,
                                           void* y2 = nullptr, const int* y2_row = nullptr, int y2_cap = 0);
+template <typename T> void launch_rmsnorm_form(hipStream_t s, const void* x, const void* g, void* y, int rows, int n, float eps, int form);
 template <typename T> void launch_rmsnorm_indexed(hipStream_t s, const void* x, const void* g, void* y, const int* src_rows, const int* tap_rows,
                                                   void* tap, int rows, int n, float eps);
 template <typename T> void launch_layernorm(hipStream_t s, const void* x, const void* g, const void* b, void* y, int rows, int n, float eps);
@@ -224,6 +229,7 @@
     const float* rope_tab;
     int T, nq, nkv, P;
     const int* dyn_pos;
+    int form = 0;
 };
 template <typename T> void launch_rope_kv(hipStream_t s, const RopeKvArgs& a);
 void launch_rope_table(hipStream_t s, float* tab, const float* inv_freq, int positions);
diff --git a/streamvln_amd/csrc/misc.hip b/streamvln_amd/csrc/misc.hip
--- a/streamvln_amd/csrc/misc.hip
+++ b/streamvln_amd/csrc/misc.hip
@@ -40,6 +40,51 @@
     if (row >= rows) return;
     T* y2r = y2 ? y2 + (size_t)min(*y2_row + row, y2_cap - 1) * n : nullptr;
     rmsnorm_row<T>(x + (size_t)row * n, g, y + (size_t)row * n, y2r, n, eps, lane);
+}
+template <typename T, int CPL>
+__global__ __launch_bounds__(256) void rmsnorm_rows_kernel(const T* x, const T* g, T* y, int rows, int n, float eps) {
+    constexpr int EPC = Elt<T>::PER_CHUNK;
+    const int lane = threadIdx.x & 63;
+    const int row = blockIdx.x * 4 + (threadIdx.x >> 6);
+    if (row >= rows) return;
+    const T* xr = x + (size_t)row * n;
+    T* yr = y + (size_t)row * n;
+    const int nch = n / EPC;
+    uint4 xc[CPL], gc[CPL];
+#pragma unroll
+    for (int u = 0; u < CPL; ++u) {
+        const int ci = lane + u * 64;
+        xc[u] = ci < nch ? *(const uint4*)(xr + (size_t)ci * EPC) : zero_chunk();
+    }
+#pragma unroll
+    for (int u = 0; u < CPL; ++u) {
+        const int ci = lane + u * 64;
+        gc[u] = ci < nch ? *(const uint4*)(g + (size_t)ci * EPC) : zero_chunk();
+    }
+    float ss = 0.0f;
+#pragma unroll
+    for (int u = 0; u < CPL; ++u) {
+        if (lane + u * 64 < nch) {
+            float f[EPC];
+            chunk_to_f32<T>(xc[u], f);
+#pragma unroll
+            for (int e = 0; e < EPC; ++e) ss += f[e] * f[e];
+        }
+    }
+    ss = wave_sum(ss);
+    const float sc = rsqrtf(ss / (float)n + eps);
+#pragma unroll
+    for (int u = 0; u < CPL; ++u) {
+        const int ci = lane + u * 64;
+        if (ci < nch) {
+            float f[EPC], gf[EPC];
+            chunk_to_f32<T>(xc[u], f);
+            chunk_to_f32<T>(gc[u], gf);
+#pragma unroll
+            for (int e = 0; e < EPC; ++e) f[e] = gf[e] * (f[e] * sc);
+            *(uint4*)(yr + (size_t)ci * EPC) = f32_to_chunk<T>(f);
+        }
+    }
 }
 template <typename T>
 __global__ __launch_bounds__(256) void rmsnorm_indexed_kernel(const T* x, const T* g, T* y, const int* src_rows, const int* tap_rows, T* tap,
@@ -87,6 +132,10 @@
     }
 }
 
+__device__ __forceinline__ void rope_pair(float x1, float x2, float c, float s, float& o1, float& o2) {
+    o1 = x1 * c - x2 * s;
+    o2 = x2 * c + x1 * s;
+}
 template <typename T>
 __global__ __launch_bounds__(256) void rope_kv_kernel(RopeKvArgs p) {
     const int i = blockIdx.x, hd = blockIdx.y * 4 + (threadIdx.x >> 6), d = threadIdx.x & 63;
@@ -98,7 +147,8 @@
     const int page = p.page_table[pos >> 6], off = pos & 63;
     if (hd < p.nq + p.nkv) {
         const float c = p.rope_tab[(size_t)pos * 128 + d], s = p.rope_tab[(size_t)pos * 128 + 64 + d];
-        const float o1 = x1 * c - x2 * s, o2 = x2 * c + x1 * s;
+        float o1, o2;
+        rope_pair(x1, x2, c, s, o1, o2);
         if (hd < p.nq) {
             row[d] = from_f32<T>(o1);
             row[d + 64] = from_f32<T>(o2);
@@ -113,6 +163,59 @@
         T* vt = (T*)p.Vpool + ((size_t)page * p.nkv + kh) * 128 * 64;
         vt[(size_t)d * 64 + off] = from_f32<T>(x1);
         vt[(size_t)(d + 64) * 64 + off] = from_f32<T>(x2);
+    }
+}
+
+template <typename T>
+__global__ __launch_bounds__(256) void rope_kv_tiled_kernel(RopeKvArgs p) {
+    constexpr int EPC = Elt<T>::PER_CHUNK, HC = 128 / EPC, HALF = HC / 2, PITCH = 128 + EPC, KC = 64 / EPC;
+    __shared__ __attribute__((aligned(16))) T vt[64 * PITCH];
+    const int hd = blockIdx.y;
+    const int lpage = (p.P >> 6) + blockIdx.x;
+    const int lo = max(p.P, lpage * 64), hi = min(p.P + p.T, lpage * 64 + 64), n = hi - lo;
+    const int page = p.page_table[lpage], o_lo = lo & 63, o_hi = o_lo + n;
+    T* base = (T*)p.qkv + (size_t)(lo - p.P) * p.ld + (size_t)hd * 128;
+    if (hd < p.nq + p.nkv) {
+        T* kdst = hd < p.nq ? nullptr : (T*)p.Kpool + (((size_t)page * p.nkv + (hd - p.nq)) * 64 + o_lo) * 128;
+        for (int e = threadIdx.x; e < n * HALF; e += 256) {
+            const int i = e / HALF, c = e - i * HALF;
+            T* row = base + (size_t)i * p.ld;
+            float x1[EPC], x2[EPC], cs[EPC], sn[EPC], o1[EPC], o2[EPC];
+            chunk_to_f32<T>(*(const uint4*)(row + c * EPC), x1);
+            chunk_to_f32<T>(*(const uint4*)(row + 64 + c * EPC), x2);
+            const float* tab = p.rope_tab + (size_t)(lo + i) * 128 + c * EPC;
+#pragma unroll
+            for (int j = 0; j < EPC; j += 4) {
+                *(float4*)(cs + j) = *(const float4*)(tab + j);
+                *(float4*)(sn + j) = *(const float4*)(tab + 64 + j);
+            }
+#pragma unroll
+            for (int j = 0; j < EPC; ++j) rope_pair(x1[j], x2[j], cs[j], sn[j], o1[j], o2[j]);
+            T* dst = kdst ? kdst + (size_t)i * 128 : row;
+            *(uint4*)(dst + c * EPC) = f32_to_chunk<T>(o1);
+            *(uint4*)(dst + 64 + c * EPC) = f32_to_chunk<T>(o2);
+        }
+        return;
+    }
+    for (int e = threadIdx.x; e < n * HC; e += 256) {
+        const int i = e / HC, c = e - i * HC;
+        *(uint4*)(vt + (o_lo + i) * PITCH + c * EPC) = *(const uint4*)(base + (size_t)i * p.ld + c * EPC);
+    }
+    __syncthreads();
+    T* vp = (T*)p.Vpool + ((size_t)page * p.nkv + (hd - p.nq - p.nkv)) * 128 * 64;
+    for (int e = threadIdx.x; e < 128 * KC; e += 256) {
+        const int d = e / KC, k0 = (e - d * KC) * EPC;
+        if (k0 + EPC <= o_lo || k0 >= o_hi) continue;
+        if (k0 >= o_lo && k0 + EPC <= o_hi) {
+            __attribute__((aligned(16))) T out[EPC];
+#pragma unroll
+            for (int j = 0; j < EPC; ++j) out[j] = vt[(k0 + j) * PITCH + d];
+            *(uint4*)(vp + (size_t)d * 64 + k0) = *(const uint4*)out;
+        } else {
+#pragma unroll
+            for (int j = 0; j < EPC; ++j)
+                if (k0 + j >= o_lo && k0 + j < o_hi) vp[(size_t)d * 64 + k0 + j] = vt[(k0 + j) * PITCH + d];
+        }
     }
 }
 
@@ -398,9 +501,25 @@
 
 
 
+constexpr int RMSNORM_ROWS_MIN = 64;
+template <typename T> void launch_rmsnorm_form(hipStream_t s, const void* x, const void* g, void* y, int rows, int n, float eps, int form) {
+    if (rows <= 0) return;
+    const int cpl = (n / Elt<T>::PER_CHUNK + 63) / 64;
+    if (form == 1 && cpl > 16) throw std::runtime_error("rmsnorm: the row does not fit the register form");
+    if (form == 2 || cpl > 16 || (form == 0 && rows < RMSNORM_ROWS_MIN)) {
+        hipLaunchKernelGGL((rmsnorm_kernel<T>), dim3((rows + 3) / 4), dim3(256), 0, s, (const T*)x, (const T*)g, (T*)y, rows, n, eps, (const int*)nullptr,
+                           (T*)nullptr, (const int*)nullptr, 0);
+        return;
+    }
+    const dim3 grid((rows + 3) / 4), block(256);
+    if (cpl <= 4) hipLaunchKernelGGL((rmsnorm_rows_kernel<T, 4>), grid, block, 0, s, (const T*)x, (const T*)g, (T*)y, rows, n, eps);
+    else if (cpl <= 8) hipLaunchKernelGGL((rmsnorm_rows_kernel<T, 8>), grid, block, 0, s, (const T*)x, (const T*)g, (T*)y, rows, n, eps);
+    else hipLaunchKernelGGL((rmsnorm_rows_kernel<T, 16>), grid, block, 0, s, (const T*)x, (const T*)g, (T*)y, rows, n, eps);
+}
 template <typename T> void launch_rmsnorm(hipStream_t s, const void* x, const void* g, void* y, int rows, int n, float eps, const int* skip,
                                           void* y2, const int* y2_row, int y2_cap) {
     if (rows <= 0) return;
+    if (!skip && !y2) { launch_rmsnorm_form<T>(s, x, g, y, rows, n, eps, 0); return; }
     hipLaunchKernelGGL((rmsnorm_kernel<T>), dim3((rows + 3) / 4), dim3(256), 0, s, (const T*)x, (const T*)g, (T*)y, rows, n, eps, skip, (T*)y2,
                        y2_row, y2_cap);
 }
@@ -415,6 +534,13 @@
     hipLaunchKernelGGL((layernorm_kernel<T>), dim3((rows + 3) / 4), dim3(256), 0, s, (const T*)x, (const T*)g, (const T*)b, (T*)y, rows, n, eps);
 }
 template <typename T> void launch_rope_kv(hipStream_t s, const RopeKvArgs& a) {
+    const bool can_tile = !a.dyn_pos && a.T >= 1 && a.ld % Elt<T>::PER_CHUNK == 0 && ((uintptr_t)a.qkv & 15) == 0;
+    if (a.form == 1 && !can_tile) throw std::runtime_error("rope_kv: the tiled form needs a host position and 16-byte aligned rows");
+    if (a.form == 1 || (a.form == 0 && can_tile && sizeof(T) == 2 && a.T >= 64)) {
+        const int pages = ((a.P + a.T - 1) >> 6) - (a.P >> 6) + 1;
+        hipLaunchKernelGGL((rope_kv_tiled_kernel<T>), dim3(pages, a.nq + 2 * a.nkv), dim3(256), 0, s, a);
+        return;
+    }
     hipLaunchKernelGGL((rope_kv_kernel<T>), dim3(a.T, (a.nq + 2 * a.nkv + 3) / 4), dim3(256), 0, s, a);
 }
 void launch_frame_hash(hipStream_t s, const float* pix, int F, size_t words_per_frame, unsigned long long* out) {
@@ -736,6 +862,7 @@
 
 #define SVLN_INST(T)                                                                                                              \
     template void launch_rmsnorm<T>(hipStream_t, const void*, const void*, void*, int, int, float, const int*, void*, const int*, int);                              \
+    template void launch_rmsnorm_form<T>(hipStream_t, const void*, const void*, void*, int, int, float, int);                                                    \
     template void launch_rmsnorm_indexed<T>(hipStream_t, const void*, const void*, void*, const int*, const int*, void*, int, int, float);                          \
     template void launch_layernorm<T>(hipStream_t, const void*, const void*, const void*, void*, int, int, float);               \
     template void launch_gather_rows_ragged<T>(hipStream_t, const int*, const void*, void*, int, int);                            \
```

Result: no change. 180.1 (median of 2 runs) (-1.0%).
